# nvaccess/NVSpeechPlayer

Hardware: AMD Instinct MI355X
Metric: audio samples/sec (whole node) at 22.05 kHz Klatt synth, batch-N utterances (higher is better)
Workload: dtype f64

## Files before the change

nvspeechplayer_amd/csrc/klatt_batchplan.h:

```cpp
#pragma once

#include <stddef.h>
#include <stdint.h>

#include <algorithm>
#include <numeric>
#include <unordered_map>
#include <utility>
#include <vector>

#include "klatt_consts.h"

namespace klatt {


template <class Meta>
inline bool list_length(const Meta* meta, long long n, uint32_t& length)
{
    unsigned long long len = 0;
    for (long long k = 0; k < n; ++k) {
        const unsigned long long m = meta[k].minSamples, f = meta[k].fadeSamples;
        len += std::max(m, f + 1) + 1;
    }
    length = len >= 0xFFFFFFFFull ? 0u : (uint32_t)len;
    return len < 0xFFFFFFFFull;
}

template <class Meta>
inline unsigned long long list_timing(const Meta* meta, long long n)
{
    unsigned long long h = 0x9E3779B97F4A7C15ull ^ (unsigned long long)n;
    for (long long k = 0; k < n; ++k) {
        h ^= ((unsigned long long)meta[k].minSamples << 32) ^ meta[k].fadeSamples ^ ((unsigned long long)(meta[k].flags & FRAME_NULL) << 63);
        h *= 0xFF51AFD7ED558CCDull; h ^= h >> 29;
    }
    return h;
}

template <class Meta, class Facts>
inline void classify_list(const Meta* meta, const Facts* facts, long long n, uint32_t& flags, unsigned char& shape)
{
    uint32_t fl = 0;
    for (long long k = 0; k < n; ++k)
        if (!(meta[k].flags & FRAME_NULL)) fl |= facts[k].flags;
    const bool finite = !(fl & FACT_NONFINITE), needsNoise = (fl & FACT_NOISE) || !finite;
    flags = needsNoise ? UTT_NEEDS_NOISE : (!(fl & FACT_NASAL) ? UTT_NO_NASAL : 0u);
    shape = finite ? (!(fl & FACT_UNBOUNDED) ? 3 : 1) : 0;
}


struct ListTable {
    std::vector<uint32_t> lens;
    std::vector<unsigned long long> timing;
    std::vector<uint32_t> flags;
    std::vector<unsigned char> shape;
    std::vector<uint32_t> weight;
    long long size() const { return (long long)flags.size(); }
    unsigned long long run_key(long long l) const { return timing[(size_t)l] ^ ((unsigned long long)lens[(size_t)l] * 0x9E3779B97F4A7C15ull); }
};

struct RouteOptions {
    int tracks = 1, direct = 1, layout = -1;
    bool fast = false;
    bool sortByLength = true;
    bool noTracks = false;
    int cus = 256;
    long long nFrames = 0;
    bool want_tracks() const { return tracks && !noTracks; }
    bool want_direct() const { return direct && layout != 0 && nFrames > 0 && nFrames < 0xFFFFFFFFll; }
    bool plans() const { return (want_tracks() || want_direct()) && nFrames > 0; }
};

constexpr long long kRunMin = 32;

struct RunShare {
    long long total = 0, inRuns = 0;
    std::unordered_map<unsigned long long, long long> runOf;
};
template <class Pred>
inline RunShare run_share(const ListTable& lists, Pred pred)
{
    RunShare s;
    for (long long l = 0; l < lists.size(); ++l)
        if (pred(l)) { s.total += lists.weight[(size_t)l]; s.runOf[lists.run_key(l)] += lists.weight[(size_t)l]; }
    for (const auto& kv : s.runOf) if (kv.second >= kRunMin) s.inRuns += kv.second;
    return s;
}

using Rerouted = std::vector<std::pair<long long, uint32_t>>;
inline Rerouted reroute_lonely_quiet(ListTable& lists, const RouteOptions& o)
{
    Rerouted rerouted;
    if (!o.plans() || o.layout != -1) return rerouted;
    auto quiet = [&](long long l) { return !(lists.flags[(size_t)l] & UTT_NEEDS_NOISE); };
    const RunShare runs = run_share(lists, quiet);
    if (runs.runOf.size() <= 1) return rerouted;
    for (long long l = 0; l < lists.size(); ++l)
        if (quiet(l) && runs.runOf.at(lists.run_key(l)) < kRunMin) {
            rerouted.emplace_back(l, lists.flags[(size_t)l]);
            lists.flags[(size_t)l] = (lists.flags[(size_t)l] | UTT_NEEDS_NOISE) & ~UTT_NO_NASAL;
        }
    return rerouted;
}

inline std::vector<unsigned char> eligible_lists(const ListTable& lists, const RouteOptions& o)
{
    std::vector<unsigned char> eligible;
    if (!o.plans()) return eligible;
    eligible.assign((size_t)lists.size(), 0);
    for (long long l = 0; l < lists.size(); ++l)
        if ((lists.flags[(size_t)l] & UTT_NEEDS_NOISE) && lists.weight[(size_t)l]) eligible[(size_t)l] = lists.shape[(size_t)l];
    return eligible;
}

inline bool tracks_pay(const ListTable& lists, const unsigned char* eligible, const unsigned char* tracked, unsigned long long trackBytes, const RouteOptions& o)
{
    if (!(o.want_direct() && o.direct == 1 && o.fast && trackBytes > (128ull << 20))) return true;
    long long direct = 0;
    const RunShare runs = run_share(lists, [&](long long l) { return tracked[l] != 0; });
    for (long long l = 0; l < lists.size(); ++l)
        if (tracked[l] && (eligible[l] & 2)) direct += lists.weight[(size_t)l];
    const long long groups = (runs.total + kLanes - 1) / kLanes;
    return !(o.sortByLength && runs.inRuns * 2 <= runs.total && direct == runs.total && groups > o.cus);
}

inline void mark_tracked(ListTable& lists, const unsigned char* tracked, const uint32_t* kinds)
{
    for (long long l = 0; l < lists.size(); ++l)
        if (tracked[l]) lists.flags[(size_t)l] |= UTT_TRACKED | (kinds[l] << kUttKindShift);
// ... 53 lines not shown
    const long long ext = width - tail;
    std::vector<uint32_t> rep((size_t)ext);
    for (long long j = 0; j < ext; ++j) rep[(size_t)j] = order[(size_t)(end - tail + j % tail)];
    order.insert(order.begin() + end, rep.begin(), rep.end());
    return ext;
}

inline void fill_sparse_wavefronts(std::vector<uint32_t>& order, long long begin, int width)
{
    const int sparse = width / 2;
    std::vector<uint32_t> live((size_t)sparse);
    for (long long w = begin; w + width <= (long long)order.size(); w += width) {
        int nLive = 0;
        for (int i = 0; i < width && nLive < sparse; ++i)
            if (order[(size_t)(w + i)] != kNoUtt) live[(size_t)nLive++] = order[(size_t)(w + i)];
        if (nLive == 0 || nLive >= sparse) continue;
        int next = 0;
        for (int i = 0; i < width; ++i)
            if (order[(size_t)(w + i)] == kNoUtt) { order[(size_t)(w + i)] = live[(size_t)next]; next = (next + 1) % nLive; }
    }
}

template <class FlagsOf>
inline LanePacking pack_lanes(long long nUtt, FlagsOf flagsOf, const uint32_t* lens, const unsigned long long* timing, bool sortByLength, int width = kLanes)
{
    LanePacking p;
    std::vector<uint32_t>& order = p.order;
    order.resize((size_t)nUtt);
    std::iota(order.begin(), order.end(), 0u);
    auto quietEnd = std::stable_partition(order.begin(), order.end(), [&](uint32_t x) { return !(flagsOf(x) & UTT_NEEDS_NOISE); });
    p.nQuiet = quietEnd - order.begin();
    auto noNasalEnd = std::stable_partition(order.begin(), quietEnd, [&](uint32_t x) { return (flagsOf(x) & UTT_NO_NASAL) != 0; });
    p.nNoNasal = noNasalEnd - order.begin();
    auto trackedEnd = std::stable_partition(quietEnd, order.end(), [&](uint32_t x) { return (flagsOf(x) & UTT_TRACKED) != 0; });
    p.nTrackedUtt = trackedEnd - quietEnd;
    p.nTracked = p.nTrackedUtt;
    auto directEnd = std::stable_partition(trackedEnd, order.end(), [&](uint32_t x) { return (flagsOf(x) & UTT_DIRECT) != 0; });
    p.nDirectSlots = directEnd - trackedEnd;
    const bool untrackedFollow = directEnd != order.end();
    if (sortByLength) {
        auto before = [&](uint32_t x, uint32_t y) { return lens[x] != lens[y] ? lens[x] > lens[y] : timing[x] < timing[y]; };
        std::stable_sort(order.begin(), noNasalEnd, before);
        std::stable_sort(noNasalEnd, quietEnd, before);
        std::stable_sort(quietEnd, trackedEnd, before);
        std::stable_sort(trackedEnd, directEnd, before);
        std::stable_sort(directEnd, order.end(), before);
        const uint32_t* const o = order.data();
        const size_t q = (size_t)p.nQuiet, t = q + (size_t)p.nTrackedUtt, d = t + (size_t)p.nDirectSlots;
        std::vector<uint32_t> tracked, direct(o + t, o + d), untracked;
        pad_runs(o + q, o + t, lens, timing, width, tracked);
        if (!tracked.empty() && t != order.size()) tracked.insert(tracked.end(), lanes_to_boundary(tracked.size(), width), kNoUtt);
        if (!direct.empty() && untrackedFollow) direct.insert(direct.end(), lanes_to_boundary(direct.size(), width), kNoUtt);
        pad_runs(o + d, o + order.size(), lens, timing, width, untracked);
        p.nTracked = (long long)tracked.size();
        p.nDirectSlots = (long long)direct.size();
        order.resize(q);
        order.insert(order.end(), tracked.begin(), tracked.end());
        order.insert(order.end(), direct.begin(), direct.end());
        order.insert(order.end(), untracked.begin(), untracked.end());
    } else if (p.nDirectSlots > 0 && (untrackedFollow || p.nTrackedUtt > 0)) {
        const size_t padT = p.nTrackedUtt > 0 ? lanes_to_boundary((size_t)p.nTrackedUtt, width) : 0;
        order.insert(order.begin() + p.nQuiet + p.nTrackedUtt, padT, kNoUtt);
        p.nTracked = p.nTrackedUtt + (long long)padT;
        if (untrackedFollow) {
            const size_t padD = lanes_to_boundary((size_t)p.nDirectSlots, width);
            order.insert(order.begin() + p.nQuiet + p.nTracked + p.nDirectSlots, padD, kNoUtt);
            p.nDirectSlots += (long long)padD;
        }
    }
    p.nNoNasalSlots = p.nNoNasal + fill_tail(order, 0, p.nNoNasal, width);
    p.nQuietSlots = p.nQuiet + (p.nNoNasalSlots - p.nNoNasal);
    p.nQuietSlots += fill_tail(order, p.nNoNasalSlots, p.nQuietSlots, width);
    const long long noisy = (long long)order.size() - p.nQuietSlots;
    if (noisy % width != 0) {
        const long long ext = width - noisy % width;
        const long long untracked = noisy - p.nTracked - p.nDirectSlots;
        if (untracked <= 0) { if (p.nDirectSlots > 0) p.nDirectSlots += ext; else p.nTracked += ext; }
        order.insert(order.end(), (size_t)ext, kNoUtt);
    }
    fill_sparse_wavefronts(order, p.nQuietSlots, width);
    return p;
}

}
```

nvspeechplayer_amd/csrc/klatt_consts.h:

```cpp
#pragma once

#include <stdint.h>

namespace klatt {

constexpr int kLanes = 64;

constexpr uint32_t FRAME_NULL = 1u;
constexpr uint32_t UTT_NEEDS_NOISE = 1u;
constexpr uint32_t UTT_NO_NASAL = 2u;
constexpr uint32_t UTT_TRACKED = 4u;
constexpr uint32_t UTT_DIRECT = 8u;
constexpr int kUttKindShift = 8;

constexpr uint32_t FACT_NOISE = 1u;
constexpr uint32_t FACT_NONFINITE = 2u;
constexpr uint32_t FACT_NASAL = 4u;
constexpr uint32_t FACT_UNBOUNDED = 8u;

}
```

nvspeechplayer_amd/csrc/klatt_device.h:

```cpp
#pragma once

#include <hip/hip_runtime.h>
#include <stdint.h>
#include <type_traits>

#include "klatt_consts.h"
#include "klatt_layout.h"
#include "klatt_math.h"

namespace klatt {

constexpr int kTile = 32;
constexpr int kTileStride = kTile * 2 + 8;
constexpr int kSlots = 45;
constexpr int kBlock = 16;
constexpr int kStateDoubles = 240;

constexpr int MODE_EXACT = 0;
constexpr int MODE_FAST = 1;

constexpr int kTrackStages = 4;
#ifndef KLATT_FLAT_LAYOUT
#define KLATT_FLAT_LAYOUT 2
#endif
__host__ __device__ constexpr uint32_t track_stage_kinds(int s)
{
    return KLATT_FLAT_LAYOUT == 2 ? (s == 0 ? 0xF04003u : s == 1 ? 0x0000FCu : s == 2 ? 0x01B000u : 0x0E0F00u)
                                  : (s == 0 ? 0xF00000u : s == 1 ? 0x00403Fu : s == 2 ? 0x01B0C0u : 0x0E0F00u);
}
__host__ __device__ constexpr uint32_t track_stage_entries(int s)
{
    return KLATT_FLAT_LAYOUT == 2 ? (s == 0 ? 8u : s == 1 ? 6u : s == 2 ? 4u : 7u) : (s == 0 ? 4u : s == 1 ? 8u : s == 2 ? 6u : 7u);
}
constexpr int kTrackAntiStage = KLATT_FLAT_LAYOUT == 2 ? 0 : 1;
__host__ __device__ inline uint32_t track_stage_slots(uint32_t mask, int s) { return (uint32_t)__builtin_popcount(mask & track_stage_kinds(s)) + (s == kTrackAntiStage ? (mask & 1u) : 0u); }
__host__ __device__ inline uint32_t track_part(uint32_t mask, uint32_t F, int s)
{
    uint32_t at = 0;
    for (int k = 0; k < s; ++k) at += track_stage_entries(k) + (F - 1u) * track_stage_slots(mask, k);
    return at;
}

struct DirectHdr {
    uint32_t fadeSamples;
    uint32_t span;
    uint32_t bits;
    uint32_t pad;
};
constexpr uint32_t kDirectBwShift = 8, kDirectClsShift = 14, kDirectAllBits = 0x3FFFFFFu;
constexpr int kDirectStages = 8;
#ifndef KLATT_DIRECT_FAST_LAYOUT
#define KLATT_DIRECT_FAST_LAYOUT 1
#endif
__host__ __device__ constexpr int direct_layout(int mode) { return mode == MODE_FAST ? KLATT_DIRECT_FAST_LAYOUT : 0; }
__host__ __device__ constexpr int direct_stage_res(int s, int L = 0)
{
    return L == 1 ? (s < 2 ? 0 : (s == 3 || s == 4) ? 3 : 2) : (s == 0 ? 0 : 2);
}
__host__ __device__ constexpr int direct_stage_gains(int s, int L = 0)
{
    return L == 1 ? (s == 0 ? 1 : s == 1 ? 3 : s == 2 ? 1 : s == 5 ? 2 : s == 6 ? 1 : s == 7 ? 2 : 0)
                  : (s == 0 ? 4 : s == 1 ? 1 : s == 5 ? 2 : s == 6 ? 1 : s == 7 ? 2 : 0);
}
__host__ __device__ constexpr int direct_stage_entries(int s, int L = 0) { return 4 * direct_stage_res(s, L) + 3 * direct_stage_gains(s, L); }
__host__ __device__ constexpr int direct_stage_first(int s, int L = 0) { int at = 0; for (int k = 0; k < s; ++k) at += direct_stage_entries(k, L); return at; }
constexpr int kDirectEntries = direct_stage_first(kDirectStages);
static_assert(direct_stage_first(kDirectStages, 1) == kDirectEntries, "both layouts hold the same kinds");
__host__ __device__ constexpr int direct_stage_kind(int s, int e, int L = 0)
{
    constexpr int k0[kDirectStages][4] = {{20, 21, 22, 23}, {0, 1, 14, -1}, {2, 3, -1, -1}, {4, 5, -1, -1}, {6, 7, -1, -1}, {8, 9, 17, 18}, {10, 11, 19, -1}, {12, 13, 15, 16}};
    constexpr int k1[kDirectStages][4] = {{20, -1, -1, -1}, {21, 22, 23, -1}, {0, 1, 14, -1}, {2, 3, 4, -1}, {5, 6, 7, -1}, {8, 9, 17, 18}, {10, 11, 19, -1}, {12, 13, 15, 16}};
    return L == 1 ? k1[s][e] : k0[s][e];
}

struct KernelArgs {
    const DirectHdr* directHdr;
    const double2* directRec;
    const uint32_t* directFirst;
    uint32_t nDirect;
    const FlatRef* flatRef;
    const SourceRef* sourceRef;
    uint32_t trackBytes;
    const double2* track;
    const double* frames;
    const FrameMeta* meta;
    const UttDesc* utt;
    const uint32_t* order;
    int16_t* pcm;
    UttResult* result;
    double* state;
    double* const* statePtrs;
    const uint32_t* control;
    long long nSlots;
    uint32_t maxSamples;
    uint32_t ringMask;
    int sampleRate;
    double sampleRateF;
    double invSampleRate;
    double negPiOverSr;
    double twoPiOverSr;
    unsigned long long* debug;
};

__device__ constexpr int kResF[kNumRes] = {13, 14, 12, 11, 10, 9, 8, 7, 25, 26, 27, 28, 29, 30};
__device__ constexpr int kResB[kNumRes] = {21, 22, 20, 19, 18, 17, 16, 15, 31, 32, 33, 34, 35, 36};
constexpr int kNumHot = 17;
__device__ constexpr int kHot[kNumHot] = {1, 2, 3, 4, 5, 6, 23, 24, 37, 38, 39, 40, 41, 42, 43, 44, 45};


__device__ __forceinline__ double div_by(double x, double b, double y)
{
    double q = x * y;
    double r = __builtin_fma(-b, q, x);
    return __builtin_fma(r, y, q);
}

__device__ __forceinline__ double frac_toward_zero(double x) { return x - __builtin_trunc(x); }

__device__ __forceinline__ double fade_value(double from, double to, double ratio)
{
    double v = from + ((to - from) * ratio);
    return (to != to) ? from : v;
}

__device__ __forceinline__ uint32_t mix32(uint32_t x)
{
    x ^= x >> 16; x *= 0x7FEB352Du; x ^= x >> 15; x *= 0x846CA68Bu; x ^= x >> 16;
    return x;
}
__device__ __forceinline__ uint32_t noise_key(uint32_t seed) { return mix32(seed ^ 0x9E3779B9u); }
__device__ __forceinline__ uint32_t noise_inc(uint32_t seed) { return (mix32(seed + 0x85EBCA6Bu) << 1) | 1u; }
constexpr uint32_t kNoiseA = 1664525u;
constexpr uint32_t kNoiseA2 = kNoiseA * kNoiseA;
__device__ __forceinline__ uint32_t noise_inc2(uint32_t inc) { return (kNoiseA + 1u) * inc; }
__device__ __forceinline__ uint32_t noise_step(uint32_t s, uint32_t inc) { return s * kNoiseA + inc; }
__device__ __forceinline__ uint32_t noise_step2(uint32_t s, uint32_t inc2) { return s * kNoiseA2 + inc2; }
__device__ __forceinline__ uint32_t noise_first(uint32_t key, uint32_t inc) { return noise_step(key, inc); }
__device__ __forceinline__ double noise_uniform(uint32_t s)
{
    const double r = (double)(s >> 1);
    return __builtin_fma(r, 0x1.00000002p-31, r * 0x1p-93);
}

template <int MODE>
__device__ __forceinline__ double dot3(double a, double x, double b, double y, double c, double z)
{
    if (MODE == MODE_FAST) return __builtin_fma(c, z, __builtin_fma(b, y, a * x));
    return a * x + b * y + c * z;
}

#ifdef KLATT_SIGNAL_F32
typedef float sig_t;
#else
typedef double sig_t;
#endif
template <int MODE>
__device__ __forceinline__ float dot3(float a, float x, float b, float y, float c, float z)
{
    return __builtin_fmaf(c, z, __builtin_fmaf(b, y, a * x));
}
__device__ __forceinline__ float fade_value(float from, float to, float ratio)
{
    float v = from + ((to - from) * ratio);
    return (to != to) ? from : v;
}

struct Coef { double a, b, c; };
enum { COEF_UNREDUCED = 0, COEF_QUADRANT_M1 = 1, COEF_UNKNOWN = 2 };
#ifndef KLATT_COLD_CALL
#define KLATT_COLD_CALL 2
#endif
struct RadCos { double rad, cs; };
#if KLATT_COLD_CALL
__device__ __attribute__((noinline)) RadCos exp_cos_reduced(double ex, double th)
{
    RadCos o;
#if KLATT_COLD_CALL == 1
    if (__builtin_fabs(ex) <= 700.0 && __builtin_fabs(th) <= 1.0e4) { o.rad = fast_exp(ex); o.cs = fast_cos(th); }
    else
#endif
    { o.rad = exp(ex); o.cs = cos(th); }
    return o;
}
#endif
// ... 451 lines not shown
```

nvspeechplayer_amd/csrc/klatt_engine.hip:

```cpp
#include "klatt_device.h"
#include "klatt_systolic.h"
#include "klatt_lanepipe.h"
#include "klatt_tracks.h"
#include "klatt_direct.h"
#include "klatt_plan.h"
#include "klatt_timeline.h"
#include "klatt_align.h"
#include "klatt_source.h"
#include "klatt_response.h"
#include "klatt_stems.h"
#include "klatt_spectrum.h"
#include "klatt_resample.h"
#include "klatt_convolve.h"
#include "klatt_filter.h"
#include "klatt_codec.h"
#include "klatt_lpc.h"
#include "klatt_tempo.h"
#include "klatt_mix.h"
#include "klatt_export.h"
#include "klatt_batchplan.h"
#include "klatt_hostpool.h"
#include "klatt_trackplan.h"
#include "klatt_live.h"

// ... 413 lines not shown
        return 0;
    };
    int rc;
    switch (mode) {
    case MODE_EXACT: rc = go(klatt_lanepipe<MODE_EXACT, CH, WPS>); break;
    case MODE_FAST: rc = go(klatt_lanepipe<MODE_FAST, CH, WPS>); break;
    default: set_error("unknown arithmetic mode %d", mode); return -1;
    }
    if (rc) return rc;
    HIP_TRY(hipGetLastError());
    return 0;
}

#ifndef KLATT_NOISY_CH
#define KLATT_NOISY_CH 8
#endif
struct GroupPlan { bool systolic; int chunk; };
GroupPlan plan_group(int layout, bool noisy, long long nUttBatch, long long nNoisyBatch, int cus)
{
    const long long groups = (nUttBatch + kLanes - 1) / kLanes + 1;
    GroupPlan p;
    p.systolic = layout != 0;
    (void)nNoisyBatch;
    p.chunk = noisy ? (groups <= cus ? 16 : 8)
                    : (groups <= cus ? 32 : 16);
    return p;
}

template <bool STREAM, bool NOISE>
int launch(const KernelArgs& a, int mode, long long nWaves, hipStream_t stream)
{
    if (nWaves <= 0) return 0;
    if (nWaves > 0x7FFFFFFF) { set_error("too many wavefronts: %lld", nWaves); return -1; }
    constexpr int ldsBytes = LdsLayout<STREAM>::kBytes;
    auto go = [&](auto kernel) -> int {
        if (ensure_lds_limit(reinterpret_cast<const void*>(kernel), ldsBytes)) return -1;
        hipLaunchKernelGGL(kernel, dim3((unsigned)nWaves), dim3(kLanes), ldsBytes, stream, a);
        return 0;
    };
    int rc;
    switch (mode) {
    case MODE_EXACT: rc = go(klatt_synthesize<MODE_EXACT, STREAM, NOISE>); break;
    case MODE_FAST: rc = go(klatt_synthesize<MODE_FAST, STREAM, NOISE>); break;
    default:
        set_error("unknown arithmetic mode %d", mode);
        return -1;
    }
    if (rc) return rc;
    HIP_TRY(hipGetLastError());
    return 0;
}

int pick_device(int device)
{
    int n = 0;
    hipError_t e = hipGetDeviceCount(&n);
    if (e != hipSuccess || n <= 0) {
        set_error_code(SPEECHPLAYER_ERR_NO_DEVICE);
        set_error("no HIP device available (%s); this engine has no CPU path", e == hipSuccess ? "count 0" : hipGetErrorString(e));
        return -1;
    }
    if (device < 0) {
        const char* env = getenv("SPEECHPLAYER_DEVICE");
        if (env) device = atoi(env);
        else if (hipGetDevice(&device) != hipSuccess) device = 0;
    }
    if (device >= n) { set_error("device %d out of range (%d devices)", device, n); return -1; }
    return device;
}

struct Batch {
    int sampleRate = 0;
    int device = 0;
    int mode = MODE_EXACT;
    int sortByLength = 1;
    int layout = -1;
    int cus = 256;
    hipStream_t stream = nullptr;
    int tracks = 1;
    long long trackBudgetMB = 4096;
    hipStream_t side[6] = {nullptr, nullptr, nullptr, nullptr, nullptr, nullptr};
    hipEvent_t forkEvent = nullptr, join[6] = {nullptr, nullptr, nullptr, nullptr, nullptr, nullptr};
    int quietLast = 1;
    long long nUtt = 0, nFrames = 0, nSlots = 0;
    long long nLists = 0, nFramesSpoken = 0;
    std::vector<long long> uttFrameStart;
    std::vector<uint32_t> uttFrames;
    bool launched = false;
    long long nQuiet = 0;
    long long nTracked = 0;
    long long nTrackedUtt = 0;
    long long nJobs = 0, trackEntries = 0;
    int directLean = -1;
    bool directAligned = false;
    int direct = 1;
    long long nDirect = 0;
    long long nDirectUtt = 0, nDirectFrames = 0;
    long long nNoNasal = 0;
    long long nNoNasalUtt = 0;
    long long totalSamples = 0, poolSamples = 0;
    std::vector<uint32_t> lens;
    std::vector<uint32_t> uttSeed;
    std::vector<long long> outStart;
    std::vector<UttResult> results;
    bool resultsFresh = false;
    DeviceBuffer<double> dFrames;
    DeviceBuffer<FrameMeta> dMeta;
    DeviceBuffer<UttDesc> dUtt;
    DeviceBuffer<uint32_t> dOrder;
    DeviceBuffer<int16_t> dPcm;
    DeviceBuffer<UttResult> dResult;
    DeviceBuffer<FlatRef> dFlatRef;
    DeviceBuffer<SourceRef> dSourceRef;
    DeviceBuffer<TrackJob> dJobs;
    DeviceBuffer<double> dShapes;
    DeviceBuffer<double2> dTrack;
    DeviceBuffer<DirectJob> dDirectJobs;
    DeviceBuffer<uint32_t> dDirectFirst;
    DeviceBuffer<DirectHdr> dDirectHdr;
    DeviceBuffer<double2> dDirectRec;
    DeviceBuffer<unsigned long long> dDebug;
    DeviceBuffer<float> dFloat;
    DeviceBuffer<unsigned long long> dDigest;
    PinnedPair bounce;
    DeviceBuffer<FrameRecord> dRecords;
    DeviceBuffer<double> dShapeTable;
    DeviceBuffer<uint32_t> dRep;
    DeviceBuffer<unsigned long long> dMismatch;
    DeviceBuffer<FrameFacts> dFacts;
    PinnedBlock hFacts;
    DeviceBuffer<int16_t> dDense;
    DeviceBuffer<long long> dDenseStart;
    std::vector<long long> denseStart;
    hipStream_t copyStream = nullptr;
    hipEvent_t denseReady = nullptr, copyDone = nullptr;
    bool copyPending = false;
    bool floatFresh = false;
    hipEvent_t inputReady = nullptr;
    DeviceBuffer<long long> dShapeIdx;
    DeviceBuffer<double> dShapeRows;
    hipEvent_t pcmReady = nullptr;
    struct ExportSlot { PinnedBlock host; DeviceBuffer<unsigned char> dev; hipEvent_t done = nullptr; bool used = false; };
    static constexpr int kExportSlots = 16;
    ExportSlot exportSlot[kExportSlots];
    unsigned exportNext = 0;
    struct SharedTable {
        hipEvent_t done = nullptr;
        bool used = false;
        int wait(hipStream_t st) { if (used) HIP_TRY(hipStreamWaitEvent(st, done, 0)); return 0; }
        int mark(hipStream_t st) { HIP_TRY(hipEventRecord(done, st)); used = true; return 0; }
    };
    std::vector<uint32_t> uttList;
    DeviceBuffer<long long> dListStart;
    DeviceBuffer<TimelineReq> dTimeline;
    hipEvent_t setDone = nullptr, setCopied = nullptr, timelineReady = nullptr;
    bool timelineFresh = false;
    ExportSlot trackSlot[kExportSlots];
    unsigned trackNext = 0;
    DeviceBuffer<double> dPitch;
    SharedTable pitchOrder;
    long long pitchBudgetMB = 256;
    DeviceBuffer<FrameLabel> dLabels;
    DeviceBuffer<uint32_t> dUnitFirst;
    std::vector<uint32_t> listUnits;
    bool hasLabels = false;
    DeviceBuffer<double> dSource;
// ... 181 lines not shown
constexpr bool kTimingOnlyBuild = false;
#endif
bool refuse_timing_only(const char* what)
{
    if (!kTimingOnlyBuild || getenv("SPEECHPLAYER_ALLOW_TIMING_ONLY_PCM")) return false;
    set_error_code(SPEECHPLAYER_ERR_ARGUMENT);
    set_error("%s: this library was built with a timing-only experiment switch; its PCM is not valid", what);
    return true;
}

long long tracked_count(const Batch* b) { return (b->tracks && b->layout != 0) ? b->nTracked : 0; }
long long direct_count(const Batch* b) { return b->nDirect; }
bool direct_lean(const Batch* b, long long nGroups)
{
    if (b->directLean >= 0) return b->directLean != 0;
    if (b->directAligned) return false;
    return b->mode == MODE_FAST ? true : nGroups > 2ll * b->cus;
}

int batch_launch(Batch* b)
{
    KernelArgs a = base_args(b->sampleRate);
    a.frames = b->dFrames.ptr; a.meta = b->dMeta.ptr; a.utt = b->dUtt.ptr;
    a.pcm = b->dPcm.ptr; a.result = b->dResult.ptr; a.state = nullptr; a.control = nullptr;
    if (wait_exports(b)) return -1;
    b->resultsFresh = false;
    b->floatFresh = false;
    b->launched = true;
#ifdef KLATT_STAMPS
    if (b->dDebug.reserve((size_t)(b->nSlots / kLpUPG + 2) * 32 * 2)) return -1;
    HIP_TRY(hipMemsetAsync(b->dDebug.ptr, 0, b->dDebug.cap * 8, b->stream));
    a.debug = b->dDebug.ptr;
#endif
    const long long nLp = lanepipe_count(b);
    const bool laneKernel = b->layout == 0;
    const long long nTr = tracked_count(b);
    const long long nDir = direct_count(b);
    const long long nNoisyHead = b->nTracked - nTr;
    const long long nNoisy = b->nSlots - b->nQuiet - b->nTracked - nDir;
    const long long nNn = laneKernel ? 0 : b->nNoNasal - nLp;
    const long long nQ = b->nQuiet - nLp - nNn;
    const int parts = (nLp > 0) + (nNn > 0) + (nQ > 0) + (nNoisy > 0) + (nNoisyHead > 0) + (nTr > 0) + (nDir > 0);
    const bool fork = parts > 1;
    if (fork) HIP_TRY(hipEventRecord(b->forkEvent, b->stream));
    int sideUsed = 0, seen = 0;
    auto next_stream = [&](bool = false) -> hipStream_t {
        if (!fork || ++seen == parts) return b->stream;
        hipStream_t st = b->side[sideUsed++];
        (void)hipStreamWaitEvent(st, b->forkEvent, 0);
        return st;
    };
    const GroupPlan plq = plan_group(b->layout, false, b->nSlots, nNoisy, b->cus);
    auto launch_quiet = [&]() -> int {
    if (nLp > 0) {
        hipStream_t st = next_stream(true);
        a.order = b->dOrder.ptr; a.nSlots = nLp;
        const long long g = (nLp + kLpUPG - 1) / kLpUPG;
        if (g <= b->cus ? launch_lanepipe<KLATT_LP_CH, 1>(a, b->mode, g, st) : launch_lanepipe<16, 2>(a, b->mode, g, st)) return -1;
    }
    if (nNn > 0) {
        hipStream_t st = next_stream(true);
        a.order = b->dOrder.ptr + nLp; a.nSlots = nNn;
        const long long g = (nNn + kLanes - 1) / kLanes;
        if (plq.chunk == 32 ? launch_systolic<false, 32, 1, false>(a, b->mode, g, st) : launch_systolic<false, 16, 2, false>(a, b->mode, g, st)) return -1;
    }
    if (nQ > 0) {
        hipStream_t st = next_stream(true);
        a.order = b->dOrder.ptr + nLp + nNn; a.nSlots = nQ;
        const long long g = (nQ + kLanes - 1) / kLanes;
        if (plq.systolic ? (plq.chunk == 32 ? launch_systolic<false, 32>(a, b->mode, g, st) : launch_systolic<false, 16>(a, b->mode, g, st))
                         : launch<false, false>(a, b->mode, g, st)) return -1;
    }
        return 0;
    };
    const bool quietLast = b->quietLast && (nTr > 0 || nDir > 0) && nNoisy == 0 && nNoisyHead == 0;
    if (!quietLast && launch_quiet()) return -1;
    if (nTr > 0) {
        hipStream_t st = next_stream();
        TrackArgs t;
        t.jobs = b->dJobs.ptr; t.nJobs = b->nJobs; t.shapes = b->dShapes.ptr; t.track = b->dTrack.ptr;
        t.negPiOverSr = a.negPiOverSr; t.twoPiOverSr = a.twoPiOverSr;
        const long long tg = b->nJobs;
        if (tg > 0x7FFFFFFF) { set_error("too many tracks: %lld", b->nJobs); return -1; }
        hipLaunchKernelGGL(klatt_tracks, dim3((unsigned)tg), dim3(kLanes * kTrackWaves), 0, st, t);
        HIP_TRY(hipGetLastError());
        a.order = b->dOrder.ptr + b->nQuiet; a.nSlots = nTr;
        a.flatRef = b->dFlatRef.ptr; a.sourceRef = b->dSourceRef.ptr; a.track = b->dTrack.ptr;
        a.trackBytes = (uint32_t)std::min<unsigned long long>(((unsigned long long)b->trackEntries + kTrackPad) * sizeof(double2), 0xFFFFFFFFull);
        const GroupPlan pl = plan_group(b->layout, true, b->nSlots, nTr + nNoisy, b->cus);
        const long long g = (nTr + kLanes - 1) / kLanes;
        if (pl.chunk == 8 ? launch_systolic<true, KLATT_FLAT_CH, KLATT_FLAT_WPS, true, false, true>(a, b->mode, g, st)
                          : launch_systolic<true, 16, 1, true, false, true>(a, b->mode, g, st)) return -1;
        a.flatRef = nullptr; a.sourceRef = nullptr; a.track = nullptr;
    }
    if (nDir > 0) {
        hipStream_t st = next_stream();
        SeedArgs sa;
        sa.jobs = b->dDirectJobs.ptr; sa.nJobs = (uint32_t)b->nDirectFrames; sa.frames = b->dFrames.ptr; sa.meta = b->dMeta.ptr;
        sa.hdr = b->dDirectHdr.ptr; sa.rec = b->dDirectRec.ptr; sa.negPiOverSr = a.negPiOverSr; sa.twoPiOverSr = a.twoPiOverSr;
        const dim3 sg((unsigned)((b->nDirectFrames + 255) / 256), (unsigned)kDirectStages);
        constexpr int kSeedLds = 14 * 257 * (int)sizeof(double2);
        if (b->mode == MODE_FAST) hipLaunchKernelGGL(klatt_seeds<MODE_FAST>, sg, dim3(256), kSeedLds, st, sa);
        else hipLaunchKernelGGL(klatt_seeds<MODE_EXACT>, sg, dim3(256), kSeedLds, st, sa);
        HIP_TRY(hipGetLastError());
        a.order = b->dOrder.ptr + b->nQuiet + b->nTracked; a.nSlots = nDir;
        a.directHdr = b->dDirectHdr.ptr; a.directRec = b->dDirectRec.ptr; a.directFirst = b->dDirectFirst.ptr; a.nDirect = (uint32_t)b->nDirectFrames;
        a.sourceRef = b->dSourceRef.ptr;
        const long long g = (nDir + kLanes - 1) / kLanes;
        if (launch_direct(a, b->mode, direct_lean(b, g), g, st)) return -1;
        a.directHdr = nullptr; a.directRec = nullptr; a.directFirst = nullptr; a.nDirect = 0; a.sourceRef = nullptr;
    }
    for (int half = 0; half < 2; ++half) {
        const long long n = half ? nNoisy : nNoisyHead;
        if (n <= 0) continue;
        hipStream_t st = next_stream();
        a.order = b->dOrder.ptr + b->nQuiet + (half ? b->nTracked + nDir : 0); a.nSlots = n;
        const GroupPlan pl = plan_group(b->layout, true, b->nSlots, nTr + nNoisy + nNoisyHead, b->cus);
        const long long g = (n + kLanes - 1) / kLanes;
        if (pl.systolic ? (pl.chunk == 8 ? launch_systolic<true, KLATT_NOISY_CH, 2>(a, b->mode, g, st) : launch_systolic<true, 16>(a, b->mode, g, st))
                        : launch<false, true>(a, b->mode, g, st)) return -1;
    }
    if (quietLast && launch_quiet()) return -1;
    for (int i = 0; i < sideUsed; ++i) {
        HIP_TRY(hipEventRecord(b->join[i], b->side[i]));
        HIP_TRY(hipStreamWaitEvent(b->stream, b->join[i], 0));
    }
    return 0;
}

constexpr size_t kLogEntries = 40960;
constexpr size_t kLogEager = 2560;

struct LogEntry {
    double p[kNumParams];
    FrameMeta meta;
    uint32_t target;
    uint32_t pad;
};
static_assert(sizeof(LogEntry) == 400, "LogEntry layout");

__global__ void __launch_bounds__(256) live_scatter(const LogEntry* __restrict__ log, uint32_t n, double* __restrict__ ringFrames,
                                                    FrameMeta* __restrict__ ringMeta)
{
    const uint32_t e = blockIdx.x * 4u + (threadIdx.x >> 6), j = threadIdx.x & 63u;
    if (e >= n) return;
    const uint32_t at = log[e].target;
    if (at == kNoTarget) return;
    if (j < (uint32_t)kNumParams) ringFrames[(size_t)at * kNumParams + j] = log[e].p[j];
    else if (j == (uint32_t)kNumParams) ringMeta[at] = log[e].meta;
}

struct LivePlace {
    FrameMeta meta;
    long long row;
    uint32_t target;
    uint32_t pad;
};
static_assert(sizeof(LivePlace) == 32, "LivePlace layout");

__global__ void __launch_bounds__(256) live_place(const double* __restrict__ frames, const LivePlace* __restrict__ place, long long n,
                                                  double* __restrict__ ringFrames, FrameMeta* __restrict__ ringMeta)
{
    const uint32_t j = threadIdx.x & 63u;
    const long long step = (long long)gridDim.x * 4;
    for (long long e = (long long)blockIdx.x * 4 + (threadIdx.x >> 6); e < n; e += step) {
        const LivePlace p = place[e];
        if (j < (uint32_t)kNumParams) ringFrames[(size_t)p.target * kNumParams + j] = p.row < 0 ? 0.0 : frames[p.row * kNumParams + j];
        else if (j == (uint32_t)kNumParams) ringMeta[p.target] = p.meta;
    }
}

struct Stream {
    int sampleRate = 0;
    int device = 0;
    int mode = MODE_EXACT;
    uint32_t seed = 0;
// ... 858 lines not shown
    begin_call();
    QueueCall q;
    q.what = "speechPlayer_queueFramesManyDevice"; q.handles = handles; q.n = nHandles; q.frameStart = frameStart; q.frames = deviceFrames;
    q.onDevice = true; q.minDur = minFrameDuration; q.fadeDur = fadeDuration; q.userIndex = userIndex; q.isNull = isNull; q.purge = purge;
    q.readyStream = static_cast<hipStream_t>(readyStream);
    return queue_frames(q);
}

int speechPlayer_handleDevice(speechPlayer_handle_t handle)
{
    begin_call();
    Stream* s = lookup(handle);
    if (!s) { set_error("speechPlayer_handleDevice: invalid handle"); return -1; }
    return s->device;
}

speechPlayer_batch_t speechPlayer_batch_create(int sampleRate, int device)
{
    begin_call();
    int dev = pick_device(device);
    if (dev < 0) return nullptr;
    Batch* b = new Batch;
    b->sampleRate = sampleRate;
    b->device = dev;
    { hipDeviceProp_t prop; if (hipGetDeviceProperties(&prop, dev) == hipSuccess && prop.multiProcessorCount > 0) b->cus = prop.multiProcessorCount; }
    bool ok = hipSetDevice(dev) == hipSuccess && hipStreamCreateWithFlags(&b->stream, hipStreamNonBlocking) == hipSuccess &&
              hipEventCreateWithFlags(&b->forkEvent, hipEventDisableTiming) == hipSuccess &&
              hipStreamCreateWithFlags(&b->copyStream, hipStreamNonBlocking) == hipSuccess &&
              hipEventCreateWithFlags(&b->denseReady, hipEventDisableTiming) == hipSuccess &&
              hipEventCreateWithFlags(&b->copyDone, hipEventDisableTiming) == hipSuccess &&
              hipEventCreateWithFlags(&b->inputReady, hipEventDisableTiming) == hipSuccess &&
              hipEventCreateWithFlags(&b->pcmReady, hipEventDisableTiming) == hipSuccess;
    for (auto& s : b->exportSlot) ok = ok && hipEventCreateWithFlags(&s.done, hipEventDisableTiming) == hipSuccess;
    for (auto& s : b->trackSlot) ok = ok && hipEventCreateWithFlags(&s.done, hipEventDisableTiming) == hipSuccess;
    for (hipEvent_t* e : {&b->setDone, &b->setCopied, &b->timelineReady, &b->pitchOrder.done, &b->sourceOrder.done, &b->resampleOrder.done, &b->bankOrder.done}) ok = ok && hipEventCreateWithFlags(e, hipEventDisableTiming) == hipSuccess;
    { const char* e = getenv("SPEECHPLAYER_TRACKS"); if (e) b->tracks = atoi(e) ? 1 : 0; }
    { const char* e = getenv("SPEECHPLAYER_DIRECT"); if (e) b->direct = std::min(2, std::max(0, atoi(e))); }
    { const char* e = getenv("SPEECHPLAYER_DIRECT_LEAN"); if (e) b->directLean = std::min(1, std::max(-1, atoi(e))); }
    for (int i = 0; i < 6 && ok; ++i)
        ok = hipStreamCreateWithFlags(&b->side[i], hipStreamNonBlocking) == hipSuccess &&
             hipEventCreateWithFlags(&b->join[i], hipEventDisableTiming) == hipSuccess;
    { const char* e = getenv("SPEECHPLAYER_QUIET_LAST"); if (e) b->quietLast = atoi(e) ? 1 : 0; }
    if (!ok) {
        set_error("cannot create a stream on device %d", dev);
        speechPlayer_batch_destroy(b);
        return nullptr;
    }
    return b;
}

void speechPlayer_batch_destroy(speechPlayer_batch_t batch)
{
    Batch* b = static_cast<Batch*>(batch);
    if (!b) return;
    (void)hipSetDevice(b->device);
    (void)sync_exports(b);
    for (auto& s : b->exportSlot) {
        if (s.done) (void)hipEventDestroy(s.done);
        s.host.release(); s.dev.release();
    }
    (void)settle_track_exports(b, true);
    for (auto& s : b->trackSlot) {
        if (s.done) (void)hipEventDestroy(s.done);
        s.host.release(); s.dev.release();
    }
    for (hipEvent_t e : {b->setDone, b->setCopied, b->timelineReady, b->pitchOrder.done, b->sourceOrder.done, b->resampleOrder.done, b->bankOrder.done}) if (e) (void)hipEventDestroy(e);
    b->dListStart.release(); b->dTimeline.release(); b->dPitch.release(); b->dLabels.release(); b->dUnitFirst.release();
    b->dSource.release(); b->dEpochs.release(); b->dEpochCount.release(); b->dResample.release(); b->dBank.release();
    if (b->inputReady) (void)hipEventDestroy(b->inputReady);
    if (b->pcmReady) (void)hipEventDestroy(b->pcmReady);
    b->dShapeIdx.release(); b->dShapeRows.release();
    if (b->stream) { (void)hipStreamSynchronize(b->stream); (void)hipStreamDestroy(b->stream); }
    for (int i = 0; i < 6; ++i) {
        if (b->side[i]) { (void)hipStreamSynchronize(b->side[i]); (void)hipStreamDestroy(b->side[i]); }
        if (b->join[i]) (void)hipEventDestroy(b->join[i]);
    }
    if (b->forkEvent) (void)hipEventDestroy(b->forkEvent);
    if (b->copyStream) { (void)hipStreamSynchronize(b->copyStream); (void)hipStreamDestroy(b->copyStream); }
    if (b->denseReady) (void)hipEventDestroy(b->denseReady);
    if (b->copyDone) (void)hipEventDestroy(b->copyDone);
    b->dDense.release(); b->dDenseStart.release(); b->dFacts.release(); b->hFacts.release();
    b->dRecords.release(); b->dShapeTable.release(); b->dRep.release(); b->dMismatch.release();
    b->dFrames.release(); b->dMeta.release(); b->dUtt.release(); b->dOrder.release(); b->dPcm.release(); b->dResult.release();
    b->dFloat.release(); b->dDebug.release(); b->dDigest.release(); b->bounce.release();
    b->dFlatRef.release(); b->dSourceRef.release(); b->dJobs.release(); b->dShapes.release(); b->dTrack.release();
    b->dDirectJobs.release(); b->dDirectFirst.release(); b->dDirectHdr.release(); b->dDirectRec.release();
    delete b;
}

int speechPlayer_batch_setOption(speechPlayer_batch_t batch, const char* name, int value)
{
    begin_call();
    Batch* b = static_cast<Batch*>(batch);
    if (!b || !name) return -1;
    if (!strcmp(name, "mode")) {
        if (value != MODE_EXACT && value != MODE_FAST) { set_error("mode %d not available", value); return -1; }
        b->mode = value;
        return 0;
    }
    if (!strcmp(name, "sort")) { b->sortByLength = value ? 1 : 0; return 0; }
    if (!strcmp(name, "quiet_last")) { b->quietLast = value ? 1 : 0; return 0; }
    if (!strcmp(name, "layout")) { b->layout = value < 0 ? -1 : (value > 2 ? 1 : value); return 0; }
    if (!strcmp(name, "tracks")) { b->tracks = value ? 1 : 0; return 0; }
    if (!strcmp(name, "track_budget_mb")) { b->trackBudgetMB = value < 0 ? 0 : value; return 0; }
    if (!strcmp(name, "direct")) { b->direct = value < 0 ? 0 : (value > 2 ? 2 : value); return 0; }
    if (!strcmp(name, "direct_lean")) { b->directLean = value < 0 ? -1 : (value ? 1 : 0); return 0; }
    if (!strcmp(name, "pitch_table_mb")) { b->pitchBudgetMB = value < 1 ? 1 : value; return 0; }
    if (!strcmp(name, "source_table_mb")) { b->sourceBudgetMB = value < 1 ? 1 : value; return 0; }
    if (!strcmp(name, "source_lane_lists")) { b->sourceLaneLists = value < 1 ? 1 : value; return 0; }
    set_error("unknown option %s", name);
    return -1;
}

struct SetInput {
    long long nLists = 0;
    const long long* listStart = nullptr;
    const speechPlayer_frame_t* frames = nullptr;
    const unsigned int* minDur = nullptr;
    const unsigned int* fadeDur = nullptr;
    const int* userIndex = nullptr;
    const unsigned char* isNull = nullptr;
    const speechPlayer_frameRecord_t* records = nullptr;
    long long nShapes = 0;
    const speechPlayer_frame_t* shapes = nullptr;
    long long nUtt = 0;
    const unsigned int* listOf = nullptr;
    const unsigned int* seeds = nullptr;
    const double* deviceFrames = nullptr;
    hipStream_t readyStream = nullptr;
    const speechPlayer_frameLabel_t* labels = nullptr;
    bool noTracks = false;
};
static_assert(sizeof(speechPlayer_frameRecord_t) == sizeof(FrameRecord), "record layout");
static_assert(sizeof(speechPlayer_frameLabel_t) == sizeof(FrameLabel), "label layout");
static_assert(SPEECHPLAYER_LABEL_GAP == kLabelGap && SPEECHPLAYER_LABEL_PUFF == kLabelPuff && SPEECHPLAYER_ALIGN_COLUMNS == kAlignColumns &&
              SPEECHPLAYER_UNIT_COLUMNS == kUnitColumns, "alignment constants");

static void batch_clear(Batch* b)
{
    b->nUtt = 0; b->nFrames = 0; b->nFramesSpoken = 0; b->nLists = 0; b->nSlots = 0; b->nQuiet = 0; b->nNoNasal = 0; b->nNoNasalUtt = 0; b->totalSamples = 0; b->poolSamples = 0;
    b->nTracked = 0; b->nTrackedUtt = 0; b->nJobs = 0; b->trackEntries = 0; b->nDirect = 0; b->nDirectUtt = 0; b->nDirectFrames = 0; b->directAligned = false;
    b->lens.clear(); b->outStart.assign(1, 0); b->results.clear(); b->resultsFresh = false; b->floatFresh = false;
    b->uttFrameStart.clear(); b->uttFrames.clear(); b->uttList.clear(); b->uttSeed.clear(); b->timelineFresh = false; b->epochFresh = false;
    b->hasLabels = false; b->listUnits.clear();
}

static int batch_set(Batch* b, const SetInput& in);

static int batch_set_guarded(const char* what, speechPlayer_batch_t batch, const SetInput& in)
{
    begin_call();
    try {
        return batch_set(static_cast<Batch*>(batch), in);
    } catch (const std::exception& e) {
        set_error("%s: %s", what, e.what());
        return -1;
    }
}

int speechPlayer_batch_setUtterances(speechPlayer_batch_t batch, long long nUtterances, const long long* frameStart,
                                     const speechPlayer_frame_t* frames, const unsigned int* minFrameDuration,
                                     const unsigned int* fadeDuration, const int* userIndex, const unsigned char* isNull,
                                     const unsigned int* noiseSeed)
{
    SetInput in;
    in.nLists = nUtterances; in.listStart = frameStart; in.frames = frames; in.minDur = minFrameDuration; in.fadeDur = fadeDuration;
    in.userIndex = userIndex; in.isNull = isNull; in.nUtt = nUtterances; in.seeds = noiseSeed;
    return batch_set_guarded("setUtterances", batch, in);
}

static bool device_range(const void* p, size_t bytes, int device, size_t align, const char* what)
{
    hipPointerAttribute_t a;
    if (hipPointerGetAttributes(&a, p) != hipSuccess) {
        (void)hipGetLastError();
        set_error("%s: %p is not memory the HIP runtime knows (host memory?)", what, p);
        return false;
    }
    if (a.type != hipMemoryTypeDevice) { set_error("%s: %p is not device memory (memory type %d)", what, p, (int)a.type); return false; }
    if (a.device != device) { set_error("%s: %p is memory of device %d, the batch's is %d", what, p, a.device, device); return false; }
    if (reinterpret_cast<uintptr_t>(p) % align) { set_error("%s: %p is not %zu-byte aligned", what, p, align); return false; }
    hipDeviceptr_t base = nullptr;
    size_t size = 0;
    if (hipMemGetAddressRange(&base, &size, const_cast<void*>(p)) != hipSuccess) {
        (void)hipGetLastError();
        set_error("%s: the allocation that holds %p is unknown to the HIP runtime", what, p);
// ... 482 lines not shown
}

static int set_upload(SetCall& c)
{
    Batch* const b = c.b;
    const SetInput& in = c.in;
    const long long nL = c.nL, nU = c.nU, nF = c.nF, pool = c.pool, nSlotsAll = (long long)c.lanes.order.size();
    const long long nTrackedUtt = c.lanes.nTrackedUtt, nDirectUtt = c.nDirectUtt;
    const TrackPlan& plan = c.plan;
    const RawVector<DirectJob>& directJobs = c.scratch.directJobs;
    if ((size_t)pool > b->dPcm.cap && sync_exports(b)) return -1;
    if (b->dFrames.reserve(std::max<size_t>((size_t)nF * kNumParams, 1)) || b->dMeta.reserve(std::max<size_t>(nF, 1)) ||
        b->dUtt.reserve(std::max<size_t>(nU, 1)) || b->dOrder.reserve(std::max<size_t>(nSlotsAll, 1)) ||
        b->dResult.reserve(std::max<size_t>(nU, 1)) || b->dPcm.reserve(std::max<size_t>(pool, 1)) || b->dListStart.reserve((size_t)nL + 1))
        return -1;
    HIP_TRY(hipMemcpyAsync(b->dListStart.ptr, c.listStart, ((size_t)nL + 1) * sizeof(long long), hipMemcpyHostToDevice, b->stream));
    if (nTrackedUtt > 0) {
        if (b->dFlatRef.reserve((size_t)nF) || b->dJobs.reserve(plan.jobs.size()) || b->dShapes.reserve(plan.shapes.size()) ||
            b->dTrack.reserve((size_t)plan.entries + kTrackPad)) return -1;
        HIP_TRY(hipMemcpyAsync(b->dShapes.ptr, plan.shapes.data(), plan.shapes.size() * sizeof(double), hipMemcpyHostToDevice, b->stream));
        HIP_TRY(hipMemcpyAsync(b->dFlatRef.ptr, c.scratch.flatRef.data(), (size_t)nF * sizeof(FlatRef), hipMemcpyHostToDevice, b->stream));
        HIP_TRY(hipMemcpyAsync(b->dJobs.ptr, plan.jobs.data(), plan.jobs.size() * sizeof(TrackJob), hipMemcpyHostToDevice, b->stream));
    }
    if (nTrackedUtt > 0 || nDirectUtt > 0) {
        if (b->dSourceRef.reserve((size_t)nF)) return -1;
    }
    if (nDirectUtt > 0) {
        const size_t nD = directJobs.size();
        if (b->dDirectJobs.reserve(nD) || b->dDirectFirst.reserve((size_t)nU) || b->dDirectHdr.reserve((size_t)kDirectStages * nD) ||
            b->dDirectRec.reserve((size_t)kDirectEntries * nD)) return -1;
        HIP_TRY(hipMemcpyAsync(b->dDirectJobs.ptr, directJobs.data(), nD * sizeof(DirectJob), hipMemcpyHostToDevice, b->stream));
        HIP_TRY(hipMemcpyAsync(b->dDirectFirst.ptr, c.directFirst.data(), (size_t)nU * sizeof(uint32_t), hipMemcpyHostToDevice, b->stream));
    }
    if (nF) {
        if (!c.earlyStarted) HIP_TRY(hipMemcpyAsync(b->dFrames.ptr, in.frames, (size_t)nF * kNumParams * sizeof(double), hipMemcpyHostToDevice, b->stream));
        if (!c.byRecords) HIP_TRY(hipMemcpyAsync(b->dMeta.ptr, c.scratch.meta.data(), (size_t)nF * sizeof(FrameMeta), hipMemcpyHostToDevice, b->stream));
    }
    if (nU) {
        HIP_TRY(hipMemcpyAsync(b->dUtt.ptr, c.utt.data(), (size_t)nU * sizeof(UttDesc), hipMemcpyHostToDevice, b->stream));
        HIP_TRY(hipMemcpyAsync(b->dOrder.ptr, c.lanes.order.data(), (size_t)nSlotsAll * sizeof(uint32_t), hipMemcpyHostToDevice, b->stream));
        HIP_TRY(hipMemsetAsync(b->dResult.ptr, 0, (size_t)nU * sizeof(UttResult), b->stream));
        if (b->dDenseStart.reserve((size_t)nU + 1)) return -1;
        HIP_TRY(hipMemcpyAsync(b->dDenseStart.ptr, c.denseStart.data(), ((size_t)nU + 1) * sizeof(long long), hipMemcpyHostToDevice, b->stream));
    }
    if (c.verify) {
        if (b->dRep.reserve((size_t)nF) || b->dMismatch.reserve(1)) return -1;
        HIP_TRY(hipMemcpyAsync(b->dRep.ptr, plan.rep.data(), (size_t)nF * sizeof(uint32_t), hipMemcpyHostToDevice, b->stream));
        HIP_TRY(hipMemsetAsync(b->dMismatch.ptr, 0xFF, sizeof(unsigned long long), b->stream));
    }
    if (in.labels) {
        if (b->dLabels.reserve(std::max<size_t>((size_t)nF, 1)) || b->dUnitFirst.reserve(std::max<size_t>((size_t)(nF + nL), 1))) return -1;
        c.copyGuard.armed = true;
        if (nF) HIP_TRY(hipMemcpyAsync(b->dLabels.ptr, in.labels, (size_t)nF * sizeof(FrameLabel), hipMemcpyHostToDevice, b->copyStream));
        if (nF + nL) HIP_TRY(hipMemcpyAsync(b->dUnitFirst.ptr, c.unitFirst.data(), (size_t)(nF + nL) * sizeof(uint32_t), hipMemcpyHostToDevice, b->copyStream));
    }
    HIP_TRY(hipStreamSynchronize(b->stream));
    if (c.copyGuard.armed) { HIP_TRY(hipStreamSynchronize(b->copyStream)); c.copyGuard.armed = false; }
    if (c.early.joinable()) c.early.join();
    if (c.earlyRc) { set_error_code(SPEECHPLAYER_ERR_HIP); set_error("set: uploading the frames failed: %s", c.earlyErr.c_str()); return -1; }
    const unsigned grid = (unsigned)std::min<long long>((nF + 255) / 256, 1 << 16);
    if (c.verify) {
        hipLaunchKernelGGL(klatt_verify_shared, dim3(grid), dim3(256), 0, b->stream, b->dFrames.ptr, b->dRep.ptr, nF, b->dMismatch.ptr);
        HIP_TRY(hipGetLastError());
        HIP_TRY(hipMemcpyAsync(&c.mismatchAt, b->dMismatch.ptr, sizeof c.mismatchAt, hipMemcpyDeviceToHost, b->stream));
    }
    if (nTrackedUtt > 0 || nDirectUtt > 0) {
        hipLaunchKernelGGL(klatt_source_refs, dim3(grid), dim3(256), 0, b->stream, b->dFrames.ptr, b->dMeta.ptr, b->dSourceRef.ptr, nF);
        HIP_TRY(hipGetLastError());
    }
    if (c.verify || nTrackedUtt > 0 || nDirectUtt > 0) HIP_TRY(hipStreamSynchronize(b->stream));
    return 0;
}

static int set_commit(SetCall& c)
{
    Batch* const b = c.b;
    const LanePacking& lanes = c.lanes;
    b->hasLabels = c.in.labels != nullptr;
    b->listUnits.swap(c.listUnits);
    b->nUtt = c.nU; b->nFrames = c.nF; b->nFramesSpoken = c.spoken; b->nLists = c.nL; b->nSlots = (long long)lanes.order.size();
    b->nNoNasalUtt = lanes.nNoNasal;
    b->nQuiet = lanes.nQuietSlots; b->nNoNasal = lanes.nNoNasalSlots;
    b->nTracked = lanes.nTrackedUtt > 0 ? lanes.nTracked : 0; b->nTrackedUtt = lanes.nTrackedUtt;
    b->nJobs = lanes.nTrackedUtt > 0 ? (long long)c.plan.jobs.size() : 0; b->trackEntries = lanes.nTrackedUtt > 0 ? (long long)c.plan.entries : 0;
    b->nDirect = c.nDirectUtt > 0 ? lanes.nDirectSlots : 0; b->nDirectUtt = c.nDirectUtt; b->nDirectFrames = (long long)c.scratch.directJobs.size();
    b->directAligned = c.nDirectUtt > 0 && c.directAligned;
    b->totalSamples = c.total; b->poolSamples = c.pool;
    b->lens.swap(c.lens); b->outStart.swap(c.outStart); b->denseStart.swap(c.denseStart);
    b->uttFrameStart.swap(c.uttFrameStart); b->uttFrames.swap(c.uttFrames); b->uttList.swap(c.uttList); b->uttSeed.swap(c.uttSeed);
    b->timelineFresh = false; b->epochFresh = false;
    HIP_TRY(hipEventRecord(b->setDone, b->stream));
    HIP_TRY(hipEventRecord(b->setCopied, b->copyStream));
    b->results.clear();
    b->resultsFresh = false;
    b->floatFresh = false;
    b->launched = false;
    return 0;
}

static int batch_set(Batch* b, const SetInput& in)
{
    if (!b || in.nLists < 0 || in.nUtt < 0 || !in.listStart) { set_error("set: bad arguments"); return -1; }
    if (in.nUtt >= 0xFFFFFFFFll || in.nLists >= 0xFFFFFFFFll) { set_error("set: too many utterances"); return -1; }
    if (!in.listOf && in.nUtt != in.nLists) { set_error("set: %lld utterances for %lld lists and no listOf", in.nUtt, in.nLists); return -1; }
    SetCall c(b, in);
    HIP_TRY(hipSetDevice(b->device));
    if (set_validate(c) || set_meta_words(c)) return -1;
    if (set_start_frames(c) || set_frame_facts(c) || set_plan(c)) return -1;
    set_direct_jobs_and_refs(c);
    set_lanes(c);
    c.verify = !c.byRecords && c.lanes.nTrackedUtt > 0 && !c.plan.rep.empty();
    if (set_upload(c)) {
        batch_clear(b);
        return -1;
    }
    c.lap("uploads");
    if (c.verify && c.mismatchAt != ~0ull) {
        const unsigned long long k = c.mismatchAt;
        if (c.early.joinable()) c.early.join();
        SetInput again = in;
        again.noTracks = true;
        const uint32_t first = c.plan.rep[(size_t)k];
        const int rc = batch_set(b, again);
        if (rc == 0) {
            set_error("set: frames %llu and %u carry one 128-bit shape hash and different values; the batch runs without tracks", k, first);
            set_error_code(SPEECHPLAYER_OK);
        }
        return rc;
    }
    return set_commit(c);
}

long long speechPlayer_batch_frames(speechPlayer_batch_t batch, long long u, speechPlayer_frame_t* frames, unsigned int* minFrameDuration,
                                    unsigned int* fadeDuration, int* userIndex, unsigned char* isNull, long long capacity)
{
    begin_call();
    Batch* b = static_cast<Batch*>(batch);
    if (!b || u < 0 || u >= b->nUtt) { set_error("batch_frames: no such utterance"); return -1; }
    HIP_TRY(hipSetDevice(b->device));
    const long long n = b->uttFrames[(size_t)u], k0 = b->uttFrameStart[(size_t)u];
    if (n > capacity || n == 0) return n;
    if (frames) HIP_TRY(hipMemcpy(frames, b->dFrames.ptr + k0 * kNumParams, (size_t)n * sizeof(speechPlayer_frame_t), hipMemcpyDeviceToHost));
    if (minFrameDuration || fadeDuration || userIndex || isNull) {
        std::vector<FrameMeta> m((size_t)n);
        HIP_TRY(hipMemcpy(m.data(), b->dMeta.ptr + k0, (size_t)n * sizeof(FrameMeta), hipMemcpyDeviceToHost));
        for (long long k = 0; k < n; ++k) {
            if (minFrameDuration) minFrameDuration[k] = m[(size_t)k].minSamples;
            if (fadeDuration) fadeDuration[k] = m[(size_t)k].fadeSamples;
            if (userIndex) userIndex[k] = m[(size_t)k].userIndex;
            if (isNull) isNull[k] = (m[(size_t)k].flags & FRAME_NULL) ? 1 : 0;
        }
    }
    return n;
}

long long speechPlayer_batch_utteranceSamples(speechPlayer_batch_t batch, long long u)
{
    Batch* b = static_cast<Batch*>(batch);
    if (!b || u < 0 || u >= b->nUtt) return -1;
    return b->lens[u];
}
long long speechPlayer_batch_lengths(speechPlayer_batch_t batch, long long* lengths, long long capacity)
{
    begin_call();
    Batch* b = static_cast<Batch*>(batch);
    if (!b) { set_error("batch_lengths: no batch"); return -1; }
// ... 657 lines not shown
    if (!b || !out) return -1;
    int n = (int)std::min<size_t>(b->dDebug.cap, (size_t)capacity);
    if (n > 0) HIP_TRY(hipMemcpy(out, b->dDebug.ptr, (size_t)n * 8, hipMemcpyDeviceToHost));
    return n;
}

int speechPlayer_batch_kernelInfo(speechPlayer_batch_t batch, int* info, int nInfo)
{
    begin_call();
    Batch* b = static_cast<Batch*>(batch);
    if (!b || !info || nInfo < 6) return -1;
    HIP_TRY(hipSetDevice(b->device));
    hipFuncAttributes fa;
    const long long nNoisy = b->nSlots - b->nQuiet, nLp = lanepipe_count(b);
    const long long nNn = b->layout == 0 ? 0 : b->nNoNasal - nLp, nQ = b->nQuiet - nLp - nNn;
    const bool lanepipe = nLp > 0 && nLp >= nQ && nLp >= nNoisy && nLp >= nNn;
    const bool nasalFree = !lanepipe && nNn > 0 && nNn >= nQ && nNn >= nNoisy;
    const bool noisy = !lanepipe && !nasalFree && nNoisy >= nQ;
    const GroupPlan pl = plan_group(b->layout, noisy, b->nSlots, nNoisy, b->cus);
    const bool fast = b->mode == MODE_FAST;
    const long long nTr = tracked_count(b);
    const long long nDir = direct_count(b);
    const bool directG = noisy && nDir > 0 && nDir >= nTr && nDir >= nNoisy - nTr - nDir;
    const bool tracked = noisy && !directG && nTr > 0 && nTr >= nNoisy - nTr - nDir;
    const void* fn;
    int ldsBytes = LdsLayout<false>::kBytes, chunk = 0, wavesPerGroup = 1;
    long long groups = (nNn + kLanes - 1) / kLanes + (nQ + kLanes - 1) / kLanes + (nNoisy + kLanes - 1) / kLanes;
    if (nasalFree) {
        if (pl.chunk == 32) { fn = fast ? (const void*)klatt_systolic<MODE_FAST, false, 32, 1, false> : (const void*)klatt_systolic<MODE_EXACT, false, 32, 1, false>; ldsBytes = SysLds<false, 32>::kBytes; }
        else { fn = fast ? (const void*)klatt_systolic<MODE_FAST, false, 16, 2, false> : (const void*)klatt_systolic<MODE_EXACT, false, 16, 2, false>; ldsBytes = SysLds<false, 16>::kBytes; }
        chunk = pl.chunk;
        wavesPerGroup = kStages;
    } else if (lanepipe) {
        const long long g = (nLp + kLpUPG - 1) / kLpUPG;
        if (g <= b->cus) { fn = fast ? (const void*)klatt_lanepipe<MODE_FAST, KLATT_LP_CH, 1> : (const void*)klatt_lanepipe<MODE_EXACT, KLATT_LP_CH, 1>; ldsBytes = LpLds<KLATT_LP_CH>::kBytes; chunk = KLATT_LP_CH; }
        else { fn = fast ? (const void*)klatt_lanepipe<MODE_FAST, 16, 2> : (const void*)klatt_lanepipe<MODE_EXACT, 16, 2>; ldsBytes = LpLds<16>::kBytes; chunk = 16; }
        wavesPerGroup = kStages;
        groups = g;
    } else if (directG) {
        if (direct_lean(b, (nDir + kLanes - 1) / kLanes)) {
            fn = fast ? (const void*)klatt_direct<MODE_FAST, kDirectLeanChunk, 4> : (const void*)klatt_direct<MODE_EXACT, kDirectLeanChunk, 4>;
            ldsBytes = DirectLds<kDirectLeanChunk>::kBytes; chunk = kDirectLeanChunk;
        } else {
            fn = fast ? (const void*)klatt_direct<MODE_FAST, kDirectChunk, 2> : (const void*)klatt_direct<MODE_EXACT, kDirectChunk, 2>;
            ldsBytes = DirectLds<kDirectChunk>::kBytes; chunk = kDirectChunk;
        }
        wavesPerGroup = kDirectStages;
    } else if (tracked) {
        if (pl.chunk == 8) { fn = fast ? (const void*)klatt_systolic<MODE_FAST, true, KLATT_FLAT_CH, KLATT_FLAT_WPS, true, false, true> : (const void*)klatt_systolic<MODE_EXACT, true, KLATT_FLAT_CH, KLATT_FLAT_WPS, true, false, true>; ldsBytes = SysLds<true, KLATT_FLAT_CH, true>::kBytes; chunk = KLATT_FLAT_CH; }
        else { fn = fast ? (const void*)klatt_systolic<MODE_FAST, true, 16, 1, true, false, true> : (const void*)klatt_systolic<MODE_EXACT, true, 16, 1, true, false, true>; ldsBytes = SysLds<true, 16, true>::kBytes; chunk = 16; }
        wavesPerGroup = kStages;
    } else if (pl.systolic) {
        if (noisy && pl.chunk == 8) { fn = fast ? (const void*)klatt_systolic<MODE_FAST, true, 8, 2> : (const void*)klatt_systolic<MODE_EXACT, true, 8, 2>; ldsBytes = SysLds<true, 8>::kBytes; }
        else if (noisy) { fn = fast ? (const void*)klatt_systolic<MODE_FAST, true, 16> : (const void*)klatt_systolic<MODE_EXACT, true, 16>; ldsBytes = SysLds<true, 16>::kBytes; }
        else if (pl.chunk == 32) { fn = fast ? (const void*)klatt_systolic<MODE_FAST, false, 32> : (const void*)klatt_systolic<MODE_EXACT, false, 32>; ldsBytes = SysLds<false, 32>::kBytes; }
        else { fn = fast ? (const void*)klatt_systolic<MODE_FAST, false, 16> : (const void*)klatt_systolic<MODE_EXACT, false, 16>; ldsBytes = SysLds<false, 16>::kBytes; }
        chunk = pl.chunk;
        wavesPerGroup = kStages;
    } else {
        fn = fast ? (noisy ? (const void*)klatt_synthesize<MODE_FAST, false, true> : (const void*)klatt_synthesize<MODE_FAST, false, false>)
                  : (noisy ? (const void*)klatt_synthesize<MODE_EXACT, false, true> : (const void*)klatt_synthesize<MODE_EXACT, false, false>);
    }
    HIP_TRY(hipFuncGetAttributes(&fa, fn));
    hipDeviceProp_t prop;
    HIP_TRY(hipGetDeviceProperties(&prop, b->device));
    info[0] = fa.numRegs;
    info[1] = ldsBytes;
    info[2] = (int)(groups * wavesPerGroup);
    info[3] = prop.multiProcessorCount;
    info[4] = (int)(prop.sharedMemPerMultiprocessor / ldsBytes);
    info[5] = (int)fa.localSizeBytes;
    if (nInfo >= 8) { info[6] = chunk; info[7] = noisy ? 1 : 0; }
    if (nInfo >= 10) { info[8] = lanepipe ? 1 : 0; info[9] = (int)std::min<long long>(nLp > 0 ? b->nNoNasalUtt : 0, 0x7FFFFFFF); }
    if (nInfo >= 12) { info[10] = nasalFree ? 1 : 0; info[11] = (int)std::min<long long>(nNn > 0 ? b->nNoNasalUtt : 0, 0x7FFFFFFF); }
    if (nInfo >= 16) {
        info[12] = (int)std::min<long long>(nTr > 0 ? b->nTrackedUtt : 0, 0x7FFFFFFF); info[13] = (int)std::min<long long>(b->nJobs, 0x7FFFFFFF);
        info[14] = (int)std::min<long long>(b->trackEntries * (long long)sizeof(double2) >> 20, 0x7FFFFFFF); info[15] = tracked ? 1 : 0;
    }
    if (nInfo >= 20) {
        info[16] = (int)std::min<long long>(b->nDirectUtt, 0x7FFFFFFF); info[17] = directG ? 1 : 0;
        info[18] = (int)std::min<long long>(b->nDirectFrames * (long long)(kDirectEntries * sizeof(double2) + kDirectStages * sizeof(DirectHdr)) >> 20, 0x7FFFFFFF);
        info[19] = 0;
    }
    return 0;
}


static long long plan_tracks_view(long long nUtterances, const long long* frameStart, const speechPlayer_frame_t* frames,
                                  const unsigned int* fadeDuration, const unsigned char* isNull, const unsigned char* eligible,
                                  long long budgetMB, const void* facts24, unsigned long long* trackOff, unsigned int* trackMask, unsigned char* tracked,
                                  unsigned long long* nEntries, long long* collisionAt, unsigned int* kinds = nullptr)
{
    begin_call();
    if (nUtterances < 0 || !frameStart || frameStart[0] != 0) { set_error("planTracks: bad arguments"); return -1; }
    for (long long u = 0; u < nUtterances; ++u)
        if (frameStart[u + 1] < frameStart[u]) { set_error("planTracks: frameStart not monotone at %lld", u); return -1; }
    const long long nF = frameStart[nUtterances];
    if (nF > 0 && (!frames || !fadeDuration)) { set_error("planTracks: bad frame arrays"); return -1; }
    std::vector<FrameMeta> meta((size_t)nF);
    for (long long k = 0; k < nF; ++k) {
        meta[k].minSamples = 0; meta[k].userIndex = -1;
        meta[k].fadeSamples = std::max(fadeDuration[k], 1u);
        meta[k].flags = (isNull && isNull[k]) ? FRAME_NULL : 0u;
    }
    std::vector<unsigned char> all;
    if (!eligible) { all.assign((size_t)nUtterances, 1); eligible = all.data(); }
    TrackPlan plan;
    std::vector<FrameFacts> own;
    const FrameFacts* facts = static_cast<const FrameFacts*>(facts24);
    if (!facts) {
        own.resize((size_t)nF);
        parallel_ranges(nF, 1 << 14, [&](long long a, long long e) { for (long long k = a; k < e; ++k) own[k] = frame_facts(reinterpret_cast<const double*>(frames + k), 1e300, 1e300); });
        facts = own.data();
    }
    plan_tracks(nUtterances, frameStart, FrameSource{frames, nullptr, nullptr}, facts, meta.data(), eligible, track_budget_entries(budgetMB), plan_hash_mask(), plan);
    if (collisionAt) *collisionAt = -1;
    for (long long k = 0; k < nF && !plan.rep.empty(); ++k) {
        const uint32_t r = plan.rep[(size_t)k];
        if (r == 0xFFFFFFFFu || (long long)r == k) continue;
        if (!shape_values_equal(reinterpret_cast<const double*>(frames + k), reinterpret_cast<const double*>(frames + r))) {
            if (collisionAt) *collisionAt = k;
            set_error("planTracks: frames %lld and %u carry one 128-bit shape hash and different values", k, r);
            return -2;
        }
    }
    for (long long k = 0; k < nF; ++k) {
        if (trackOff) trackOff[k] = plan.ref[k].off;
        if (trackMask) trackMask[k] = plan.ref[k].mask;
    }
    for (long long u = 0; u < nUtterances; ++u) {
        if (tracked) tracked[u] = plan.tracked[u];
        if (kinds) kinds[u] = plan.tracked[u] ? plan.kinds[u] : 0u;
        if (!plan.tracked[u])
            for (long long k = frameStart[u]; k < frameStart[u + 1]; ++k) { if (trackOff) trackOff[k] = 0; if (trackMask) trackMask[k] = 0; }
    }
    if (nEntries) *nEntries = plan.entries;
    return (long long)plan.jobs.size();
}

long long speechPlayer_planTracks(long long nUtterances, const long long* frameStart, const speechPlayer_frame_t* frames,
                                  const unsigned int* fadeDuration, const unsigned char* isNull, const unsigned char* eligible,
                                  long long budgetMB, unsigned long long* trackOff, unsigned int* trackMask, unsigned char* tracked,
                                  unsigned long long* nEntries)
{
    try {
        return plan_tracks_view(nUtterances, frameStart, frames, fadeDuration, isNull, eligible, budgetMB, nullptr, trackOff, trackMask, tracked, nEntries, nullptr);
    } catch (const std::exception& e) { set_error("planTracks: %s", e.what()); return -1; }
}

long long speechPlayer_planTracksFacts(long long nUtterances, const long long* frameStart, const speechPlayer_frame_t* frames,
                                       const unsigned int* fadeDuration, const unsigned char* isNull, const unsigned char* eligible,
                                       long long budgetMB, const void* facts24, unsigned long long* trackOff, unsigned int* trackMask,
                                       unsigned char* tracked, unsigned long long* nEntries, long long* collisionAt)
{
    try {
        return plan_tracks_view(nUtterances, frameStart, frames, fadeDuration, isNull, eligible, budgetMB, facts24, trackOff, trackMask, tracked, nEntries, collisionAt);
    } catch (const std::exception& e) { set_error("planTracksFacts: %s", e.what()); return -1; }
}

long long speechPlayer_planTrackKinds(long long nUtterances, const long long* frameStart, const speechPlayer_frame_t* frames,
                                      const unsigned int* fadeDuration, const unsigned char* isNull, const unsigned char* eligible,
                                      long long budgetMB, unsigned long long* trackOff, unsigned int* trackMask, unsigned char* tracked,
                                      unsigned long long* nEntries, unsigned int* kinds)
{
    try {
        return plan_tracks_view(nUtterances, frameStart, frames, fadeDuration, isNull, eligible, budgetMB, nullptr, trackOff, trackMask, tracked, nEntries, nullptr, kinds);
    } catch (const std::exception& e) { set_error("planTrackKinds: %s", e.what()); return -1; }
}

void speechPlayer_internal_parallel(long long n, long long grain, void (*fn)(void* ctx, long long a, long long e), void* ctx)
{
    if (n <= 0 || !fn) return;
    parallel_ranges(n, grain, [&](long long a, long long e) { fn(ctx, a, e); });
}

long long speechPlayer_frameFacts(const speechPlayer_frame_t* frames, long long nFrames, int sampleRate, int onDevice, void* facts24)
{
    begin_call();
    if (nFrames < 0 || (nFrames > 0 && (!frames || !facts24)) || sampleRate <= 0) { set_error("frameFacts: bad arguments"); return -1; }
    const double maxBw = 690.0 * sampleRate / M_PI, maxF = 9900.0 * sampleRate / (2.0 * M_PI);
    FrameFacts* const out = static_cast<FrameFacts*>(facts24);
    if (!onDevice) {
        parallel_ranges(nFrames, 1 << 13, [&](long long a, long long e) { for (long long k = a; k < e; ++k) out[k] = frame_facts(reinterpret_cast<const double*>(frames + k), maxF, maxBw); });
        return nFrames;
    }
    if (nFrames == 0) return 0;
    DeviceBuffer<double> dF;
    DeviceBuffer<FrameFacts> dO;
    struct Release { DeviceBuffer<double>& a; DeviceBuffer<FrameFacts>& b; ~Release() { a.release(); b.release(); } } release{dF, dO};
    if (dF.reserve((size_t)nFrames * kNumParams) || dO.reserve((size_t)nFrames)) return -1;
    HIP_TRY(hipMemcpy(dF.ptr, frames, (size_t)nFrames * kNumParams * sizeof(double), hipMemcpyHostToDevice));
    const unsigned grid = (unsigned)std::min<long long>((nFrames + 255) / 256, 1 << 16);
    hipLaunchKernelGGL(klatt_frame_facts, dim3(grid), dim3(256), 0, nullptr, dF.ptr, dO.ptr, nFrames, maxF, maxBw);
    HIP_TRY(hipGetLastError());
    HIP_TRY(hipMemcpy(out, dO.ptr, (size_t)nFrames * sizeof(FrameFacts), hipMemcpyDeviceToHost));
    return nFrames;
}

long long speechPlayer_planDirect(long long nUtterances, const long long* frameStart, const unsigned char* isNull,
                                  unsigned int* from, unsigned int* to, unsigned int* flags)
{
    begin_call();
    if (nUtterances < 0 || !frameStart || frameStart[0] != 0) { set_error("planDirect: bad arguments"); return -1; }
    for (long long u = 0; u < nUtterances; ++u)
        if (frameStart[u + 1] < frameStart[u]) { set_error("planDirect: frameStart not monotone at %lld", u); return -1; }
    const long long nF = frameStart[nUtterances];
    if (nF >= 0xFFFFFFFFll) { set_error("planDirect: too many frames"); return -1; }
    std::vector<FrameMeta> meta((size_t)nF);
    for (long long k = 0; k < nF; ++k) { meta[k].minSamples = 0; meta[k].fadeSamples = 1; meta[k].userIndex = -1; meta[k].flags = (isNull && isNull[k]) ? FRAME_NULL : 0u; }
    std::vector<DirectJob> jobs;
    jobs.reserve((size_t)nF);
    for (long long u = 0; u < nUtterances; ++u) walk_fade_ends(frameStart[u], frameStart[u + 1], meta.data(), jobs);
    for (long long k = 0; k < nF; ++k) {
        if (from) from[k] = jobs[(size_t)k].from;
        if (to) to[k] = jobs[(size_t)k].to;
        if (flags) flags[k] = jobs[(size_t)k].flags;
    }
    return nF;
}

long long speechPlayer_planTimeline(long long nUtterances, const long long* frameStart, const unsigned int* minFrameDuration,
                                    const unsigned int* fadeDuration, long long* firstSample, long long* length)
{
    begin_call();
    if (nUtterances < 0 || !frameStart || frameStart[0] != 0) { set_error("planTimeline: bad arguments"); return -1; }
    for (long long u = 0; u < nUtterances; ++u)
        if (frameStart[u + 1] < frameStart[u]) { set_error("planTimeline: frameStart not monotone at %lld", u); return -1; }
    const long long nF = frameStart[nUtterances];
    if (nF > 0 && (!minFrameDuration || !fadeDuration)) { set_error("planTimeline: no durations"); return -1; }
    for (long long u = 0; u < nUtterances; ++u) {
        long long S = 0;
        for (long long k = frameStart[u]; k < frameStart[u + 1]; ++k) {
            if (firstSample) firstSample[k] = S;
            FrameMeta m;
            m.minSamples = minFrameDuration[k]; m.fadeSamples = std::max(fadeDuration[k], 1u);
            S += timeline_span(m);
        }
        if (length) length[u] = S;
    }
    return nF;
}

long long speechPlayer_batch_timeline(speechPlayer_batch_t batch, long long u, long long* firstSample, int* userIndex, long long capacity)
{
    begin_call();
    Batch* b = static_cast<Batch*>(batch);
    if (!b || u < 0 || u >= b->nUtt) { set_error("batch_timeline: no such utterance"); return -1; }
    HIP_TRY(hipSetDevice(b->device));
    const long long n = b->uttFrames[(size_t)u], k0 = b->uttFrameStart[(size_t)u];
    if (n > capacity || (!firstSample && !userIndex)) return n;
    std::vector<FrameMeta> m((size_t)n);
    if (n) HIP_TRY(hipMemcpy(m.data(), b->dMeta.ptr + k0, (size_t)n * sizeof(FrameMeta), hipMemcpyDeviceToHost));
    long long S = 0;
    for (long long k = 0; k < n; ++k) {
        if (firstSample) firstSample[k] = S;
        if (userIndex) userIndex[k] = m[(size_t)k].userIndex;
        S += timeline_span(m[(size_t)k]);
    }
    if (firstSample) firstSample[n] = S;
    return n;
}

static int export_output(Batch* b, const char* what, void* deviceOut, long long elements, size_t elSize)
{
    HIP_TRY(hipSetDevice(b->device));
    if (!deviceOut) { set_error("%s: no output buffer", what); return -1; }
    return device_range(deviceOut, (size_t)elements * elSize, b->device, elSize, what) ? 0 : -1;
}

static int export_synthesised(const Batch* b, const char* what)
{
    if (!b->launched) set_error("%s: the batch has not been synthesised since it was set", what);
    return b->launched ? 0 : -1;
}

static int step_request(const char* what, long long& hop, long long& phase, long long rowStride)
{
    if (hop <= 0 || phase < 0) { set_error("%s: hop %lld, phase %lld", what, hop, phase); return -1; }
// ... 2048 lines not shown
```

nvspeechplayer_amd/csrc/klatt_plan.h:

```cpp
#pragma once

#include <stdint.h>
#include <string.h>

#include "klatt_consts.h"
#include "klatt_layout.h"
#if defined(__HIPCC__)
#include "klatt_device.h"
#endif

namespace klatt {

struct FrameFacts {
    unsigned long long h0, h1;
    uint32_t flags;
    uint32_t pad;
};

KLATT_LAYOUT_HD inline bool fact_finite(double v)
{
    unsigned long long w;
    memcpy(&w, &v, 8);
    return (w & 0x7FF0000000000000ull) != 0x7FF0000000000000ull;
}
KLATT_LAYOUT_HD inline double fact_abs(double v) { return v < 0 ? -v : v; }
KLATT_LAYOUT_HD constexpr unsigned long long fact_key(int n)
{
    unsigned long long z = (unsigned long long)(n + 1) * 0x9E3779B97F4A7C15ull;
    z = (z ^ (z >> 30)) * 0xBF58476D1CE4E5B9ull;
    z = (z ^ (z >> 27)) * 0x94D049BB133111EBull;
    return z ^ (z >> 31);
}
KLATT_LAYOUT_HD inline unsigned long long fact_fold(unsigned long long a, unsigned long long c)
{
#if defined(__HIP_DEVICE_COMPILE__)
    return (__umul64hi(a, c) ^ (a * c)) + a + ((c << 32) | (c >> 32));
#else
    const unsigned __int128 m = (unsigned __int128)a * c;
    return ((unsigned long long)(m >> 64) ^ (unsigned long long)m) + a + ((c << 32) | (c >> 32));
#endif
}

KLATT_LAYOUT_HD inline uint32_t pitch_flags(double p0, double p46)
{
    uint32_t fl = 0;
    if (!fact_finite(p0) || !fact_finite(p46)) fl |= 2u;
    if (!(fact_abs(p0) <= 1e30) || !(fact_abs(p46) <= 1e30)) fl |= 4u;
    return fl;
}
KLATT_LAYOUT_HD inline uint32_t shape_flags(const double* p, double maxF, double maxBw)
{
    uint32_t fl = 0;
    if (p[3] != 0.0 || p[6] != 0.0 || p[24] != 0.0) fl |= 1u;
    bool finite = true;
    for (int i = 1; i < kNumParams - 1; ++i) finite = finite && fact_finite(p[i]);
    if (!finite) fl |= 2u;
    for (int i = 25; i <= 30; ++i)
        if (!(fact_abs(p[i]) <= 1e6) || !(p[i + 6] >= 0.0) || !(p[i + 6] <= 1e6)) fl |= 1u;
    if (p[23] != 0.0 || !(p[21] >= 1.0) || !(p[22] >= 0.0) || !(p[21] <= 1e6) || !(p[22] <= 1e6) ||
        !(fact_abs(p[13]) <= 1e6) || !(fact_abs(p[14]) <= 1e6) || !(fact_abs(p[5]) <= 1e30) || !(fact_abs(p[44]) <= 1e30))
        fl |= 4u;
    bool inRange = true;
    for (int i = 7; i <= 14; ++i) inRange = inRange && (fact_abs(p[i]) <= maxF) && (p[i + 8] >= 0.0) && (p[i + 8] <= maxBw);
    for (int i = 25; i <= 30; ++i) inRange = inRange && (fact_abs(p[i]) <= maxF) && (p[i + 6] >= 0.0) && (p[i + 6] <= maxBw);
    if (!inRange) fl |= 8u;
    return fl;
}
KLATT_LAYOUT_HD inline bool shape_values_equal(const double* a, const double* c)
{
    bool same = true;
    for (int i = 1; i < kNumParams - 1; ++i) {
        unsigned long long x, y;
        memcpy(&x, &a[i], 8); memcpy(&y, &c[i], 8);
        same = same && x == y;
    }
    return same;
}

KLATT_LAYOUT_HD inline FrameFacts frame_facts(const double* p, double maxF, double maxBw)
{
    FrameFacts o;
    const uint32_t fl = shape_flags(p, maxF, maxBw) | pitch_flags(p[0], p[46]);
    unsigned long long x = 0x9E3779B97F4A7C15ull, y = 0xC2B2AE3D27D4EB4Full;
#if defined(__HIPCC__)
#pragma unroll
#endif
    for (int i = 0; i < 46; i += 2) {
        unsigned long long w0, w1 = 0;
        memcpy(&w0, &p[1 + i], 8);
        if (i + 1 < kShapeValues) memcpy(&w1, &p[2 + i], 8);
        x ^= fact_fold(w0 ^ fact_key(2 * i), w1 ^ fact_key(2 * i + 1));
        y ^= fact_fold(w0 ^ fact_key(2 * i + 100), w1 ^ fact_key(2 * i + 101));
    }
    x ^= x >> 32; x *= 0xD6E8FEB86659FD93ull; x ^= x >> 32;
    y ^= y >> 31; y *= 0xBF58476D1CE4E5B9ull; y ^= y >> 29;
    o.h0 = x; o.h1 = y; o.flags = fl; o.pad = 0;
    return o;
}

#if defined(__HIPCC__)
__global__ void __launch_bounds__(256) klatt_frame_facts(const double* __restrict__ frames, FrameFacts* __restrict__ out, long long nFrames, double maxF, double maxBw)
{
    const long long stride = (long long)gridDim.x * blockDim.x;
    for (long long k = (long long)blockIdx.x * blockDim.x + threadIdx.x; k < nFrames; k += stride) {
        double p[kNumParams];
        const double* src = frames + k * kNumParams;
#pragma unroll
        for (int i = 0; i < kNumParams; ++i) p[i] = src[i];
        out[k] = frame_facts(p, maxF, maxBw);
    }
}

struct FrameRecord {
    double voicePitch, endVoicePitch;
    uint32_t shape;
    uint32_t minSamples, fadeSamples;
    int32_t userIndex;
};
constexpr uint32_t kRecordSilence = 0xFFFFFFFFu;
static_assert(sizeof(FrameRecord) == 32, "FrameRecord layout");

__global__ void __launch_bounds__(256) klatt_expand_frames(const FrameRecord* __restrict__ records, const double* __restrict__ shapes,
                                                           double* __restrict__ frames, FrameMeta* __restrict__ meta, long long nFrames)
{
    constexpr int kTileFrames = 64, kTilePairs = kTileFrames * kNumParams / 2;
    __shared__ FrameRecord rec[kTileFrames];
    const long long nTiles = (nFrames + kTileFrames - 1) / kTileFrames;
    for (long long tile = blockIdx.x; tile < nTiles; tile += gridDim.x) {
        const long long k0 = tile * kTileFrames;
        const int n = (int)((nFrames - k0) < (long long)kTileFrames ? (nFrames - k0) : (long long)kTileFrames);
        __syncthreads();
        if ((int)threadIdx.x < n) {
            const FrameRecord r = records[k0 + threadIdx.x];
            rec[threadIdx.x] = r;
            FrameMeta m;
            m.minSamples = r.minSamples;
            m.fadeSamples = r.fadeSamples > 1u ? r.fadeSamples : 1u;
            m.userIndex = r.userIndex;
            m.flags = r.shape == kRecordSilence ? FRAME_NULL : 0u;
            meta[k0 + threadIdx.x] = m;
        }
        __syncthreads();
        auto value = [&](int j) -> double {
            const int f = j / kNumParams, p = j - f * kNumParams;
// ... 30 lines not shown
```

nvspeechplayer_amd/csrc/klatt_systolic.h:

```cpp
#pragma once

#include <type_traits>

#include "klatt_device.h"

namespace klatt {

#ifndef KLATT_UNROLL
#define KLATT_UNROLL 8
#endif
#ifndef KLATT_MINWAVES
#define KLATT_MINWAVES 1
#endif
#ifndef KLATT_PAIR
#define KLATT_PAIR 1
#endif
#ifndef KLATT_NOISY_RUNS
#define KLATT_NOISY_RUNS 0
#endif
#ifndef KLATT_FADE_TIGHT
#define KLATT_FADE_TIGHT 1
#endif
#ifndef KLATT_NOISY_TIGHT
#define KLATT_NOISY_TIGHT 1
#endif
#define KLATT_STR2(x) #x
#define KLATT_STR(x) KLATT_STR2(x)

#ifndef KLATT_FLAT_EXHAUSTIVE
#define KLATT_FLAT_EXHAUSTIVE 1
#endif
constexpr int kStages = 4;
#ifndef KLATT_FLAT_SOURCE
#define KLATT_FLAT_SOURCE 1
#endif

template <bool NOISE, int CH, bool FLAT = false, int SPLIT = 0>
struct SysLds {
    static constexpr int MOVED = SPLIT & 3;
    static constexpr bool NP0 = (SPLIT >> 2) != 0;
    static constexpr int kBufs = 2;
    static constexpr int kBufsX = 2;
    static constexpr int kBufBytes = CH * kLanes * (FLAT ? (int)sizeof(sig_t) : 8);
    static constexpr int kPipeBytes = kBufs * kBufBytes;
    static constexpr int kNumPipes = NOISE ? 4 : 3;
    static constexpr int kPipeO = kBufsX * kBufBytes;
    static constexpr int kTileOff = kPipeO + (kNumPipes - 1) * kPipeBytes;
    static constexpr int kRowBase = kTileOff + kLanes * kTileStride;
    static constexpr int kRowCount = kRowBase + kLanes * 8;
    static constexpr int kMaxLen = kRowCount + kLanes * 4;
    static constexpr int kSync = kMaxLen + 16;
    static constexpr int kFrames = kSync + 32;
    static constexpr int kParams0 = (FLAT && KLATT_FLAT_SOURCE) ? 0 : (NP0 ? 12 : 7), kParams1 = FLAT ? 0 : (NOISE ? (NP0 ? 0 : 5) + 2 * (3 + MOVED) : 7), kParams2 = FLAT ? 0 : (NOISE ? 14 - 2 * MOVED : 6), kParams3 = FLAT ? 0 : (NOISE ? 14 : 5);
    static constexpr int kFrames1 = kFrames + 1 * kParams0 * kLanes * 8;
    static constexpr int kFrames2 = kFrames1 + 2 * kParams1 * kLanes * 8;
    static constexpr int kFrames3 = kFrames2 + 2 * kParams2 * kLanes * 8;
    static constexpr int kBytes = kFrames3 + 2 * kParams3 * kLanes * 8;
};

template <int NPARAM, int NRES, bool NWREG = false>
struct StageFrame {
    double* oldL;
    double* nwL;
    double nwR[NWREG && NPARAM > 0 ? NPARAM : 1];
    __device__ __forceinline__ double getNew(int k) const { return NWREG ? nwR[k] : nwL[k * kLanes]; }
    __device__ __forceinline__ void setNew(int k, double v) { if (NWREG) nwR[k] = v; else nwL[k * kLanes] = v; }
    double cur[NPARAM > 0 ? NPARAM : 1];
    double ra[NRES > 0 ? NRES : 1], rb[NRES > 0 ? NRES : 1], rc[NRES > 0 ? NRES : 1];
    double z1[NRES > 0 ? NRES : 1], z2[NRES > 0 ? NRES : 1];
    double invFade;
    uint32_t cnt, oldMin, newMin, newFade, nextFrame, resMask, parMask, produced;
    bool hasNew, oldNull, newNull, done;
};

struct PitchState {
    double cur0, old0, new0, oldInc, newInc;
};

template <int NPARAM, int NRES, bool NWREG>
__device__ __forceinline__ void stage_frame_init(StageFrame<NPARAM, NRES, NWREG>& f, bool live, unsigned char* region, int lane)
{
    f.oldL = reinterpret_cast<double*>(region) + lane;
    f.nwL = f.oldL + NPARAM * kLanes;
#pragma unroll
    for (int k = 0; k < NPARAM; ++k) { f.oldL[k * kLanes] = 0.0; f.setNew(k, 0.0); f.cur[k] = 0.0; }
#pragma unroll
    for (int r = 0; r < NRES; ++r) { f.ra[r] = 0.0; f.rb[r] = 2.0; f.rc[r] = -1.0; f.z1[r] = 0.0; f.z2[r] = 0.0; }
    f.invFade = 1.0;
    f.cnt = 0; f.oldMin = 0; f.newMin = 0; f.newFade = 1; f.nextFrame = 0; f.resMask = 0; f.parMask = 0; f.produced = 0;
    f.hasNew = false; f.oldNull = true; f.newNull = false; f.done = !live;
}

template <int NPARAM_, int NRES_, int GAIN_, bool PITCH_, bool ANTI0_, bool INLINE_COEF_ = false>
struct StageDesc {
    static constexpr int NPARAM = NPARAM_, NRES = NRES_, GAIN = GAIN_;
    static constexpr bool PITCH = PITCH_, ANTI0 = ANTI0_, INLINE_COEF = INLINE_COEF_;
};

struct StageCtx {
    const KernelArgs& A;
    const UttDesc& d;
    const double* myFrames;
    const FrameMeta* myMeta;
    uint32_t ringOff, ringMask;
    const FlatRef* myFlat;
    const SourceRef* mySrc;
    bool lone = false;
    double* loneLds = nullptr;
};
constexpr int kLoneLdsPerStage = 12288;
#ifndef KLATT_STREAM_SPLIT
#define KLATT_STREAM_SPLIT 5
#endif
#ifndef KLATT_LONE_SPLIT
#define KLATT_LONE_SPLIT 7
// ... 547 lines not shown
                        }
                    }
                    if (K::RUNS && !K::LONE && !forceGeneral()) {
                        const bool fad = f.hasNew;
                        const uint32_t rem = f.done ? 0xFFFFFFFFu : (fad ? f.newFade - f.cnt : (f.oldMin > f.cnt ? f.oldMin - f.cnt : 0u));
                        const bool anyFad = __any(!f.done && fad), anySteady = __any(!f.done && !fad);
                        int n = 0;
                        if (!(anyFad && anySteady) && !__any(!f.done && fad && f.cnt == 0u) && !(anyFad && nan_target_live(f))) {
                            const int cap = lim - i;
#pragma unroll
                            for (int st = CH; st >= 1; st >>= 1)
                                if (n + st <= cap && __all(rem >= (uint32_t)(n + st))) n += st;
                        }
                        if (n >= 2) {
                            int kr = anyFad ? 1 : 0;
                            bool lerpR = false, gainOnlyR = false;
                            uint32_t wResR = 0;
                            if (kr == 1) {
                                lerpR = __any(!f.done && f.parMask != 0u);
                                gainOnlyR = D::GAIN >= 0 && !__any(!f.done && (f.parMask & ~(1u << GI)) != 0u);
                                wResR = wave_or_bits<(D::NRES > 0 ? D::NRES : 1)>(f.done ? 0u : f.resMask);
                                if (!D::PITCH && !lerpR && wResR == 0u) kr = 0;
                            }
                            if (!f.done) {
                                if (kr == 0) {
#pragma nounroll
                                    for (int j = i; j < i + n; ++j) body(c, j, true, K::PRE ? preIn(c, j) : 0.0);
                                    f.cnt += (uint32_t)n;
                                    steadyDone(n);
                                } else {
#pragma nounroll
                                    for (int j = i; j < i + n; ++j) {
                                        f.cnt++;
                                        stage_fade<D, MODE, true>(f, ps, X.A, RF, RB, lerpR, wResR, gainOnlyR);
                                        body(c, j, false, 0.0);
                                    }
                                    fadeDone(n);
                                }
                            }
                            i += n;
                            continue;
                        }
                    }
                    if (K::DELAY) {
                        const bool hold = delay > 0u;
                        const bool wasDone = f.done;
                        if (hold) { delay--; f.done = true; }
                        const bool emit = stage_advance<D, MODE>(f, ps, lastIndex, P, RF, RB, X);
                        if (hold) f.done = wasDone;
                        gen(c, i, emit);
                    } else if (K::CACHE) {
                        if (!cached) {
#pragma unroll
                            for (int k = 0; k < D::NPARAM; ++k) { co[k] = f.oldL[k * kLanes]; cn[k] = f.getNew(k); }
                            cached = true;
                        }
                        bool anyEvent = false;
                        const bool emit = stage_advance<D, MODE>(f, ps, lastIndex, P, RF, RB, X, co, cn, &anyEvent);
                        if (anyEvent) cached = false;
                        gen(c, i, emit);
                    } else {
                        const bool emit = stage_advance<D, MODE>(f, ps, lastIndex, P, RF, RB, X);
                        if (K::LONE) loneValid = false;
                        gen(c, i, emit);
                    }
                    ++i;
                }
            }
            perChunk();
        }
        STAMP_WORKED();
        STAGE_SYNC();
        STAMP_SYNCED();
    }
#ifdef KLATT_STAMPS
    if (X.A.debug && (threadIdx.x & (kLanes - 1)) == 0) {
        unsigned long long* o = X.A.debug + (blockIdx.x * 4 + stampSlot) * 8;
        o[0] = st.work; o[1] = st.wait; o[2] = st.n[0]; o[3] = st.n[1]; o[4] = st.n[2]; o[5] = st.c[0]; o[6] = st.c[1]; o[7] = st.c[2];
    }
#endif
    (void)stampSlot;
}

template <int STAGE_, int NRES_, int NGAIN_, bool ANTI0_, uint32_t USUAL_ = 0, uint32_t USUAL2_ = 0, class R_ = sig_t>
struct FlatDesc {
    using R = R_;
    static constexpr int STAGE = STAGE_;
    static constexpr int NRES = NRES_, NGAIN = NGAIN_, NE = NRES_ + NGAIN_;
    static constexpr bool ANTI0 = ANTI0_;
    static constexpr uint32_t USUAL = USUAL_, USUAL2 = USUAL2_;
};

struct BarrierSync {
    __device__ __forceinline__ void begin(int) const {}
    __device__ __forceinline__ void end(int) const { __syncthreads(); }
    __device__ __forceinline__ void idle() const { __syncthreads(); }
};

#ifndef KLATT_MIX_UNROLL
#define KLATT_MIX_UNROLL 4
#endif
template <int E> using KindTag = std::integral_constant<int, E>;
typedef unsigned int flat_u4 __attribute__((ext_vector_type(4)));
typedef unsigned int flat_u2 __attribute__((ext_vector_type(2)));
typedef double flat_d2 __attribute__((ext_vector_type(2)));
template <class FD>
struct FlatState2 {
    static constexpr int NR = FD::NRES > 0 ? FD::NRES : 1;
    using R = typename FD::R;
    R ra[NR], rb[NR], rc[NR], z1[NR], z2[NR];
    R cur[2 * FD::NGAIN > 0 ? 2 * FD::NGAIN : 1];
    uint32_t idx[FD::NE], stride[FD::NE];
    uint32_t startAt, left, next, nFrames, length, produced;
    FlatRef nextRef;
    uint32_t wmask;
    bool live;
};
template <class R> struct ResPre { R a, p1, p2; };
template <class T> __device__ __forceinline__ void flat_pin(T v) { asm volatile("" :: "v"(v) : "memory"); }
template <class R> __device__ __forceinline__ void flat_pin(const ResPre<R>& q) { asm volatile("" :: "v"(q.a), "v"(q.p1), "v"(q.p2) : "memory"); }
template <int NE>
__device__ __forceinline__ uint32_t flat2_wave_kinds(uint32_t flags, bool live, const int* GE)
{
    const uint32_t mine = live ? (flags >> kUttKindShift) : 0u;
    uint32_t w = 0;
#pragma unroll
    for (int e = 0; e < NE; ++e) w |= __any((mine >> GE[e]) & 1u) ? (1u << e) : 0u;
    return w;
}
template <class FD>
__device__ __forceinline__ void flat2_init(FlatState2<FD>& f, bool live, const UttDesc& d, const StageCtx& X, const int* GE)
{
#pragma unroll
    for (int r = 0; r < FD::NRES; ++r) { f.ra[r] = 0; f.rb[r] = 2; f.rc[r] = -1; f.z1[r] = 0; f.z2[r] = 0; }
#pragma unroll
    for (int k = 0; k < 2 * FD::NGAIN; ++k) f.cur[k] = 0;
#pragma unroll
    for (int e = 0; e < FD::NE; ++e) { f.idx[e] = 0; f.stride[e] = 0; }
    f.live = live && d.length > 0u;
    f.nFrames = d.nFrames; f.length = d.length; f.next = 0; f.left = 0; f.produced = 0;
    const bool any = live && d.nFrames > 0u;
    f.startAt = any ? 1u : 0xFFFFFFFFu;
    f.nextRef = FlatRef{0u, 0u, 1u, 0u};
    if (any) f.nextRef = X.myFlat[0];
    f.wmask = (uint32_t)__builtin_amdgcn_readfirstlane((int)flat2_wave_kinds<FD::NE>(d.flags, live, GE));
}
template <class FD>
__device__ __forceinline__ void flat2_switch(FlatState2<FD>& f, const StageCtx& X, const int* GE)
{
    const FlatRef p = f.nextRef;
    const uint32_t part = p.off + track_part(p.mask, p.fadeSamples, FD::STAGE);
    const uint32_t nMove = track_stage_slots(p.mask, FD::STAGE), hdr = track_stage_entries(FD::STAGE) - nMove;
    uint32_t moving = 0, still = 0;
#pragma unroll
    for (int e = 0; e < FD::NE; ++e) {
        const bool moves = (p.mask >> GE[e]) & 1u;
        f.idx[e] = (part + (moves ? hdr + moving : still)) * 16u;
        f.stride[e] = moves ? nMove * 16u : 0u;
        const uint32_t w = GE[e] == 0 ? 2u : 1u;
        moving += moves ? w : 0u; still += moves ? 0u : w;
    }
    f.left = nMove ? p.fadeSamples : 1u;
    f.next++;
    const bool more = f.next < f.nFrames;
    f.startAt = more ? f.startAt + p.span : 0xFFFFFFFFu;
#pragma unroll
    for (int e = 0; e < FD::NE; ++e) { flat_pin(f.idx[e]); flat_pin(f.stride[e]); }
    flat_pin(f.left); flat_pin(f.startAt);
    f.nextRef = X.myFlat[more ? f.next : f.nFrames - 1u];
}
template <class FD, uint32_t SET, bool ALLROWS = false>
struct FlatMid {
    FlatState2<FD>& f;
    __amdgpu_buffer_rsrc_t rsrc;
    bool has;
    template <class... T>
    __device__ __forceinline__ void operator()(T... firstHalf) const
    {
        using R = typename FD::R;
        (flat_pin(firstHalf), ...);
        if (ALLROWS || has) {
#pragma unroll
            for (int e = 0; e < FD::NE; ++e) {
                if (!(SET & (1u << e))) continue;
                const uint32_t off = f.idx[e];
                const flat_d2 v = __builtin_bit_cast(flat_d2, __builtin_amdgcn_raw_buffer_load_b128(rsrc, off, 0, 0));
                if (e < FD::NRES) {
                    f.rb[e < FD::NRES ? e : 0] = (R)v.x; f.rc[e < FD::NRES ? e : 0] = (R)v.y;
                    if (FD::ANTI0 && e == 0) f.ra[0] = (R)__builtin_bit_cast(double, __builtin_amdgcn_raw_buffer_load_b64(rsrc, off + 16u, 0, 0));
                } else {
                    const int g = e < FD::NRES ? 0 : e - FD::NRES;
                    f.cur[2 * g] = (R)v.x; f.cur[2 * g + 1] = (R)v.y;
                }
                f.idx[e] = off + f.stride[e];
            }
        }
    }
};
struct NoMid { template <class... T> __device__ __forceinline__ void operator()(T...) const {} };
template <int MODE, bool DERIVE, class R>
__device__ __forceinline__ ResPre<R> res_pre(R ra, R rb, R rc, R z1, R z2)
{
    ResPre<R> p;
    p.a = DERIVE ? (R)((R)1 - rb - rc) : ra;
    if (MODE == MODE_FAST || !std::is_same<R, double>::value) { p.p1 = rb; p.p2 = rc; }
    else { p.p1 = rb * z1; p.p2 = rc * z2; }
    return p;
}
template <int MODE, class R>
__device__ __forceinline__ R res_post(const ResPre<R>& p, R in, R& z1, R& z2)
{
    R y;
    if (MODE == MODE_FAST || !std::is_same<R, double>::value) y = dot3<MODE>(p.a, in, p.p1, z1, p.p2, z2);
    else y = p.a * in + p.p1 + p.p2;
    z2 = z1; z1 = y;
    return y;
}

template <class FD, int CH, class FBody, class FChunk, class FSync = BarrierSync>
__device__ __forceinline__ void flat2_loop(int depth, int nIter, int nChunks, int stampSlot, FlatState2<FD>& f, const StageCtx& X, const int* GE, FBody body, FChunk perChunk,
                                           const FSync& sync = FSync{})
{
#ifdef KLATT_STAMPS
    Stamps st;
#endif
    using R = typename FD::R;
    uint32_t staleG = 0;
    const __amdgpu_buffer_rsrc_t rsrc = __builtin_amdgcn_make_buffer_rsrc(const_cast<double2*>(X.A.track), 0, (int)X.A.trackBytes, 0x00020000);
    for (int iter = 0; iter < nIter; ++iter) {
        STAMP_BEGIN();
        STAMP_IDLE();
        const int c = iter - depth;
        const bool inRange = c >= 0 && c < nChunks;
        if (inRange) {
            sync.begin(c);
            const uint32_t t0 = (uint32_t)c * (uint32_t)CH, t1 = t0 + (uint32_t)CH;
            if (f.length <= t0) f.live = false;
            const bool busy = f.left > 0u || f.startAt <= t1;
// ... 57 lines not shown
                        if (tn == f.startAt) flat2_switch<FD>(f, X, GE);
                    }
                    const bool has = ALLROWS || f.left > 0u;
                    body(c, i, setTag, FlatMid<FD, SET, ALLROWS>{f, rsrc, has});
                    if (!ALLROWS && has) f.left--;
                }
                if (ALLROWS) f.left = f.left > (uint32_t)CH ? f.left - (uint32_t)CH : 0u;
            };
            constexpr uint32_t ALL = (1u << FD::NE) - 1u;
            const bool usual = FD::USUAL != 0u && FD::USUAL != ALL && c != 0 && (f.wmask & ~FD::USUAL) == 0u;
            const bool allRows = usual && __all(!f.live || (f.left >= (uint32_t)CH && f.startAt > t1));
            if (allRows) mixedChunk(std::integral_constant<uint32_t, FD::USUAL>{}, std::true_type{});
            else if (usual) mixedChunk(std::integral_constant<uint32_t, FD::USUAL>{}, std::false_type{});
            else mixedChunk(std::integral_constant<uint32_t, ALL>{}, std::false_type{});
            f.produced = f.length < t1 ? f.length : t1;
            perChunk();
        }
        STAMP_WORKED();
        if (inRange) sync.end(c); else sync.idle();
        STAMP_SYNCED();
    }
#ifdef KLATT_STAMPS
    if (X.A.debug && (threadIdx.x & (kLanes - 1)) == 0) {
        unsigned long long* o = X.A.debug + (blockIdx.x * 4 + stampSlot) * 8;
        o[0] = st.work; o[1] = st.wait; o[2] = st.n[0]; o[3] = st.n[1]; o[4] = st.n[2]; o[5] = st.c[0]; o[6] = st.c[1]; o[7] = st.c[2];
    }
#endif
    (void)stampSlot;
}

template <int MODE, bool NOISE, int CH, int WPS = KLATT_MINWAVES, bool NASAL = true, bool STREAM = false, bool FLAT = false, bool LONE = false>
__global__ void __launch_bounds__(kLanes * kStages, WPS) klatt_systolic(const KernelArgs A)
{
    static_assert(!LONE || STREAM, "LONE: a live handle pulled alone");
    static_assert(NASAL || !NOISE, "only quiet launches have a nasal-free instantiation");
    static_assert(NOISE || !STREAM, "live handles take the noisy instantiation");
    static_assert(!FLAT || (NOISE && !STREAM), "tracks: noisy batch launches");
    constexpr int SPLIT = stream_split<STREAM, WPS, LONE>();
    constexpr int MOVED = SPLIT & 3;
    using L = SysLds<NOISE, CH, FLAT, SPLIT>;
    static_assert(SPLIT != 3, "eight resonators in the head stage: not built");
    constexpr int kChunk = CH;
    extern __shared__ __attribute__((aligned(16))) unsigned char lds[];
    using PipeT = typename std::conditional<FLAT, sig_t, double>::type;
    PipeT* const pipeX = reinterpret_cast<PipeT*>(lds);
    PipeT* const pipeO = reinterpret_cast<PipeT*>(lds + L::kPipeO);
    PipeT* const pipeA = reinterpret_cast<PipeT*>(lds + L::kPipeO + L::kPipeBytes);
    PipeT* const pipeB = reinterpret_cast<PipeT*>(lds + L::kPipeO + (NOISE ? 2 : 1) * L::kPipeBytes);
    constexpr int nbuf_pipeX = L::kBufsX, nbuf_pipeO = L::kBufs, nbuf_pipeA = L::kBufs, nbuf_pipeB = L::kBufs;
    (void)nbuf_pipeX; (void)nbuf_pipeO; (void)nbuf_pipeA; (void)nbuf_pipeB;
    unsigned char* const tile = lds + L::kTileOff;
    long long* const rowBase = reinterpret_cast<long long*>(lds + L::kRowBase);
    uint32_t* const rowCount = reinterpret_cast<uint32_t*>(lds + L::kRowCount);
    uint32_t* const maxLenP = reinterpret_cast<uint32_t*>(lds + L::kMaxLen);

    const int lane = threadIdx.x & (kLanes - 1);
    const int wave = __builtin_amdgcn_readfirstlane(threadIdx.x >> 6);
    const long long slot = (long long)blockIdx.x * kLanes + lane;
    const uint32_t u = (slot < A.nSlots) ? A.order[slot] : 0xFFFFFFFFu;
    const bool live = (u != 0xFFFFFFFFu);

    UttDesc d;
    d.frameStart = 0; d.outStart = 0; d.nFrames = 0; d.seed = 0; d.flags = 0; d.length = 0;
    if (live) d = A.utt[u];
    const FrameWindow fw = frame_window(A, d);
    const StageCtx X{A, d, A.frames + fw.base * kNumParams, A.meta + fw.base, fw.off, fw.mask,
                     FLAT ? A.flatRef + d.frameStart : nullptr, FLAT ? A.sourceRef + d.frameStart : nullptr, LONE,
                     LONE ? reinterpret_cast<double*>(lds + L::kBytes + wave * kLoneLdsPerStage) : nullptr};
    const uint32_t nkey = noise_key(d.seed), ninc = noise_inc(d.seed), ninc2 = noise_inc2(ninc);
    constexpr int FINAL = NOISE ? 2 : 3;
#ifndef KLATT_PRELOAD
#define KLATT_PRELOAD 1
#endif
    constexpr bool kPre = !NOISE && KLATT_PRELOAD;

    uint32_t* const stageMaskP = maxLenP + 1;
    uint32_t* const syncP = reinterpret_cast<uint32_t*>(lds + L::kSync);
    if (threadIdx.x == 0) { *maxLenP = 0; *stageMaskP = 0; }
    if (threadIdx.x < 8) syncP[threadIdx.x] = 0;
    __syncthreads();
    int cand = wave;
    if (KLATT_PAIR && WPS == 2 && (NOISE || !NASAL)) {
        const uint32_t hw = __builtin_amdgcn_s_getreg((4 << 0) | (0 << 6) | (31 << 11));
        cand = (int)((((hw >> 4) & 3u) + ((hw & 1u) ? 2u : 0u)) & 3u);
    }
    if (wave == 0) atomicMax(maxLenP, d.length);
    if (lane == 0) atomicOr(stageMaskP, 1u << cand);
    __syncthreads();
    const int stage = __builtin_amdgcn_readfirstlane((*stageMaskP == 0xFu) ? cand : wave);
    if (stage == FINAL) { rowBase[lane] = d.outStart; rowCount[lane] = 0; }
    const uint32_t maxLen = *maxLenP;
    const int nChunks = (int)((maxLen + kChunk - 1) / kChunk);
    const int nIter = nChunks + (NOISE ? 2 : 3);
    const int fullChunks = STREAM ? (int)(A.maxSamples / (uint32_t)kChunk) : nChunks;
    double* const streamState = (STREAM && live) ? (A.statePtrs ? A.statePtrs[u] : A.state + (size_t)u * kStateDoubles) : nullptr;
    const bool streamPurge = STREAM && live && A.control && (A.control[u] & 1u);
#define PIPE(p, c, i) (p)[(((nbuf_##p) == 2 ? ((c) & 1) : ((c) % (nbuf_##p))) * kChunk + (i)) * kLanes + lane]
    using KSrc = LoopKnobs<false, (!NOISE || KLATT_NOISY_RUNS), false, STREAM, NOISE, KLATT_UNROLL, LONE, (STREAM && WPS == 1 && !LONE)>;
    using KFil = LoopKnobs<kPre, (!NOISE || KLATT_NOISY_RUNS), false, STREAM, NOISE, KLATT_UNROLL, LONE, (STREAM && WPS == 1 && !LONE)>;
    uint32_t noDelay = 0;
    auto never = [&]() __attribute__((always_inline)) { return false; };
    auto noBegin = [&](int) __attribute__((always_inline)) { return false; };
    auto noAlt = [&](int) __attribute__((always_inline)) {};
    auto noAltSample = [&](int, int, double) __attribute__((always_inline)) {};
    auto noFadeAlt = [&](int, bool, bool) __attribute__((always_inline)) { return false; };
    auto nothing = [&](int) __attribute__((always_inline)) {};
    auto noChunk = [&]() __attribute__((always_inline)) {};

    auto make_sync = [&](auto, auto, auto, int, int, int) __attribute__((always_inline)) { return BarrierSync{}; };
    using I0 = std::integral_constant<int, 0>; using I1 = std::integral_constant<int, 1>; using I2 = std::integral_constant<int, 2>;
    if (FLAT && KLATT_FLAT_SOURCE && stage == 0) {
        if constexpr (FLAT) {
#if KLATT_FLAT_LAYOUT == 2
            using FD = FlatDesc<0, 2, 5, true, 0, 0, double>;
            constexpr int GE[7] = {0, 1, 14, 20, 21, 22, 23};
            constexpr int CB = 2;
            constexpr uint32_t kUsualS0 = 0x67u, kAllS0 = 0x7Fu, kVibBit = 8u;
            constexpr bool kHead = true;
#else
            using FD = FlatDesc<0, 0, 4, false, 0, 0, double>;
            constexpr int GE[4] = {20, 21, 22, 23};
            constexpr int CB = 0;
            constexpr uint32_t kUsualS0 = 0xCu, kAllS0 = 0xFu, kVibBit = 1u;
            constexpr bool kHead = false;
#endif
            bool staleNP = false;
            FlatState2<FD> f;
            flat2_init<FD>(f, live, d, X, GE);
            PitchState ps;
            ps.cur0 = 0.0; ps.old0 = 0.0; ps.new0 = 0.0; ps.oldInc = 0.0; ps.newInc = 0.0;
            double pitchPhase = 0.0, vibPhase = 0.0, aspNoise = 0.0, invFade = 1.0, nfD = 1.0;
            uint32_t noiseSt = noise_first(nkey, ninc), cntF = 0, nfU = 0;
            uint32_t fadeEndAt = 0xFFFFFFFFu;
            int32_t lastIndex = -1;
            bool oldNull = true, newNull = false;
            SourceRef nextSrc{0.0, 0.0, 1.0, -1, 0u};
            if (live && d.nFrames > 0u) nextSrc = X.mySrc[0];
            auto source = [&](bool waveVib, auto setTag, const auto& mid) __attribute__((always_inline)) -> double {
                constexpr uint32_t SET = decltype(setTag)::value;
                double vib = 1.0;
                if (waveVib) {
                    const double vs = f.cur[CB + 1];
                    const double adv = frac_toward_zero(div_by(vs, A.sampleRateF, A.invSampleRate) + vibPhase);
                    vibPhase = (vs != 0.0) ? adv : vibPhase;
                    vib = (sin(vibPhase * 6.283185307179586) * 0.06 * f.cur[CB + 0]) + 1.0;
                }
                const double turbGain = f.cur[CB + 2], openQ = f.cur[CB + 3], voiceAmp = f.cur[CB + 4], aspAmp = f.cur[CB + 5], preGain = f.cur[CB + 6];
                pitchPhase = frac_toward_zero(div_by(ps.cur0 * vib, A.sampleRateF, A.invSampleRate) + pitchPhase);
                double voice = (pitchPhase * 2.0) - 1.0;
                aspNoise = noise_uniform(noiseSt) + 0.75 * aspNoise;
                noiseSt = noise_step2(noiseSt, ninc2);
                double asp = aspNoise * 0.2;
                double turb = asp * turbGain;
                turb = (pitchPhase >= openQ) ? turb : turb * 0.01;
                voice += turb;
                voice *= voiceAmp;
                asp *= aspAmp;
                const double src = asp + voice;
                const double out = (src * preGain) * 0.5;
                if constexpr (kHead) {
                    const ResPre<double> q0 = res_pre<MODE, false>(f.ra[0], f.rb[0], f.rc[0], f.z1[0], f.z2[0]);
                    const ResPre<double> q1 = res_pre<MODE, ((SET >> 1) & 1u) != 0u>(f.ra[1], f.rb[1], f.rc[1], f.z1[1], f.z2[1]);
                    const double caNP = f.cur[0];
                    mid(out, q0, q1, caNP);
                    double zin = f.z1[0];
                    const double n0 = res_post<MODE>(q0, out, zin, f.z2[0]);
                    f.z1[0] = out;
                    const double np = res_post<MODE>(q1, n0, f.z1[1], f.z2[1]);
                    return fade_value(out, np, caNP);
                } else {
                    mid(out);
                    return out;
                }
            };
            auto vib_live = [&]() __attribute__((always_inline)) -> bool { return f.cur[CB + 0] != 0.0 || f.cur[CB + 1] != 0.0 || vibPhase != vibPhase; };
            const __amdgpu_buffer_rsrc_t rsrc = __builtin_amdgcn_make_buffer_rsrc(const_cast<double2*>(A.track), 0, (int)A.trackBytes, 0x00020000);
#ifdef KLATT_STAMPS
            Stamps st;
#endif
            const auto sync = make_sync(std::integral_constant<int, L::kBufsX>{}, I0{}, I1{}, 0, 0, 0);
            for (int iter = 0; iter < nIter; ++iter) {
                STAMP_BEGIN();
                STAMP_IDLE();
                const int c = iter;
                int lastChunk = -1;
                if (c < nChunks) {
                    sync.begin(c);
                    lastChunk = c;
                    const uint32_t t0 = (uint32_t)c * (uint32_t)CH, t1 = t0 + (uint32_t)CH;
                    if (f.length <= t0) f.live = false;
                    const bool busy = f.left > 0u || f.startAt <= t1 || cntF < nfU || fadeEndAt < t1 || vib_live();
                    STAMP_KIND(__any(busy) ? -1 : 0);
                    if (!__any(busy)) {
                        uint32_t run = f.live ? (f.startAt - t0 - 1u) / (uint32_t)CH : 0xFFFFFFFFu;
#pragma unroll
                        for (int m = 32; m >= 1; m >>= 1) { const uint32_t o = (uint32_t)__shfl_xor((int)run, m, kLanes); run = o < run ? o : run; }
                        run = (uint32_t)__builtin_amdgcn_readfirstlane((int)run);
                        const uint32_t room = (uint32_t)(nChunks - c);
                        run = run < room ? run : room;
                        run = run < 1u ? 1u : run;
                        int cc = c;
                        if (kHead && staleNP) { f.ra[1] = 1.0 - f.rb[1] - f.rc[1]; staleNP = false; }
                        for (uint32_t q = 0; q < run; ++q) {
                            if (f.live) {
#pragma unroll
                                for (int i = 0; i < CH; ++i) { ps.cur0 += ps.oldInc; PIPE(pipeX, cc, i) = source(false, std::integral_constant<uint32_t, 0u>{}, NoMid{}); }
                                ps.old0 = ps.cur0;
                            }
                            if (q + 1 < run) { STAMP_WORKED(); sync.end(cc); STAMP_SYNCED(); STAMP_BEGIN(); ++iter; ++cc; sync.begin(cc); lastChunk = cc; }
                        }
                    } else {
                        auto mixedChunk = [&](auto setTag, auto allFadeTag) __attribute__((always_inline)) {
                        constexpr uint32_t SET = decltype(setTag)::value;
                        constexpr bool ALLFADE = decltype(allFadeTag)::value;
                        const bool vibChunk = (SET & kVibBit) != 0u || __any(vib_live());
                        staleNP = true;
#pragma unroll KLATT_MIX_UNROLL
                        for (int i = 0; i < CH; ++i) {
                            const uint32_t t = t0 + (uint32_t)i;
                            const bool deq = !ALLFADE && t + 1u == f.startAt;
                            if (!ALLFADE && __any(deq)) {
                                if (deq) {
                                    const SourceRef m = nextSrc;
                                    const uint32_t nf = f.nextRef.fadeSamples;
                                    newNull = (m.flags & FRAME_NULL) != 0;
                                    ps.new0 = newNull ? ps.cur0 : m.pitch;
                                    ps.newInc = newNull ? 0.0 : m.pitchInc;
                                    if (!newNull && oldNull) ps.old0 = m.pitch;
                                    oldNull = newNull;
                                    if (m.userIndex != -1) lastIndex = m.userIndex;
                                    nfD = (double)nf; nfU = nf;
                                    ps.new0 += ps.newInc * nfD;
                                    invFade = m.invFade;
                                    cntF = 0;
                                    fadeEndAt = t + nf + 1u;
                                    flat_pin(ps.new0); flat_pin(ps.newInc); flat_pin(ps.old0); flat_pin(invFade); flat_pin(lastIndex); flat_pin(oldNull);
                                    flat2_switch<FD>(f, X, GE);
                                    nextSrc = X.mySrc[f.next < f.nFrames ? f.next : f.nFrames - 1u];
                                }
                            }
                            if (ALLFADE) {
                                cntF++;
                                ps.cur0 = fade_value(ps.old0, ps.new0, div_by((double)cntF, nfD, invFade));
                            } else {
                            const bool fad = !deq && cntF < nfU;
                            const bool ending = !deq && !fad && t == fadeEndAt;
                            const bool glide = !deq && !fad && !ending;
                            const uint32_t cn = cntF + 1u;
                            const double ratio = div_by((double)cn, nfD, invFade);
                            const double fv = fade_value(ps.old0, ps.new0, ratio);
                            const double gv = ps.cur0 + ps.oldInc;
                            ps.cur0 = fad ? fv : (glide ? gv : ps.cur0);
                            ps.old0 = ending ? ps.new0 : (glide ? gv : ps.old0);
                            ps.oldInc = ending ? ps.newInc : ps.oldInc;
                            cntF = fad ? cn : cntF;
                            fadeEndAt = ending ? 0xFFFFFFFFu : fadeEndAt;
                            }
                            const bool waveVib = vibChunk && __any(vib_live());
                            const bool has = f.left > 0u;
                            PIPE(pipeX, c, i) = source(waveVib, setTag, FlatMid<FD, SET>{f, rsrc, has});
                            if (has) f.left--;
                        }
                        };
                        const bool usual = c != 0 && (f.wmask & ~kUsualS0) == 0u;
                        const bool allFade = usual && !__any(vib_live()) && __all(!f.live || (cntF + (uint32_t)CH <= nfU && f.startAt > t1));
                        if (allFade) mixedChunk(std::integral_constant<uint32_t, kUsualS0>{}, std::true_type{});
                        else if (usual) mixedChunk(std::integral_constant<uint32_t, kUsualS0>{}, std::false_type{});
                        else mixedChunk(std::integral_constant<uint32_t, kAllS0>{}, std::false_type{});
                    }
                }
                STAMP_WORKED();
                if (lastChunk >= 0) sync.end(lastChunk); else sync.idle();
                STAMP_SYNCED();
            }
#ifdef KLATT_STAMPS
            if (A.debug && lane == 0) {
                unsigned long long* o = A.debug + (blockIdx.x * 4 + 0) * 8;
                o[0] = st.work; o[1] = st.wait; o[2] = st.n[0]; o[3] = st.n[1]; o[4] = st.n[2]; o[5] = st.c[0]; o[6] = st.c[1]; o[7] = st.c[2];
            }
#endif
            if (live) {
                UttResult res;
                res.produced = d.length; res.framesTaken = f.next; res.lastIndex = lastIndex; res.drained = 1u;
                A.result[u] = res;
            }
        }
    } else if (stage == 0) {
        constexpr bool NP0 = (SPLIT >> 2) != 0;
        using D = StageDesc<NP0 ? 12 : 7, NP0 ? 2 : 0, 6, true, NP0, NP0>;
        constexpr int P[12] = {1, 2, 3, 4, 5, 6, 44, 13, 21, 14, 22, 23};
        constexpr int RF[2] = {7, 9}, RB[2] = {8, 10};
        StageFrame<D::NPARAM, D::NRES, true> f;
        PitchState ps;
        stage_frame_init(f, live, lds + L::kFrames, lane);
        ps.cur0 = 0.0; ps.old0 = 0.0; ps.new0 = 0.0; ps.oldInc = 0.0; ps.newInc = 0.0;
        double pitchPhase = 0.0, vibPhase = 0.0, aspNoise = 0.0;
        uint32_t noiseSt = noise_first(nkey, ninc);
        int32_t lastIndex = -1;
        bool vibFrames = false;
        constexpr int GR0[2] = {0, 1};
        if (STREAM && live) {
            if (streamState[239] != 0.0) {
                pitchPhase = streamState[208]; vibPhase = streamState[209]; aspNoise = streamState[210];
                lastIndex = (int32_t)streamState[220]; noiseSt = (uint32_t)streamState[221];
            }
            stage_state_load<D>(f, &ps, streamState, P, RF, RB, GR0, streamPurge);
            vibFrames = f.oldL[0] != 0.0 || f.oldL[kLanes] != 0.0 || f.getNew(0) != 0.0 || f.getNew(1) != 0.0;
        }

        auto source = [&](bool waveVib) __attribute__((always_inline)) -> double {
            double vib = 1.0;
            if (waveVib) {
                const double vs = f.cur[1];
                const double adv = frac_toward_zero(div_by(vs, A.sampleRateF, A.invSampleRate) + vibPhase);
                vibPhase = (vs != 0.0) ? adv : vibPhase;
                vib = (sin(vibPhase * 6.283185307179586) * 0.06 * f.cur[0]) + 1.0;
            }
            pitchPhase = frac_toward_zero(div_by(ps.cur0 * vib, A.sampleRateF, A.invSampleRate) + pitchPhase);
            double voice = (pitchPhase * 2.0) - 1.0;
            double src;
            if (NOISE) {
                aspNoise = noise_uniform(noiseSt) + 0.75 * aspNoise;
                noiseSt = noise_step2(noiseSt, ninc2);
                double asp = aspNoise * 0.2;
                double turb = asp * f.cur[2];
                turb = (pitchPhase >= f.cur[3]) ? turb : turb * 0.01;
                voice += turb;
                voice *= f.cur[4];
                asp *= f.cur[5];
                src = asp + voice;
            } else {
                src = voice * f.cur[4];
            }
            const double x = (src * f.cur[6]) * 0.5;
            if (!NP0) return x;
            const double n0 = dot3<MODE>(f.ra[0], x, f.rb[0], f.z1[0], f.rc[0], f.z2[0]);
            f.z2[0] = f.z1[0]; f.z1[0] = x;
            const double np = resonate<MODE>(f.z1[NP0 ? 1 : 0], f.z2[NP0 ? 1 : 0], f.ra[NP0 ? 1 : 0], f.rb[NP0 ? 1 : 0], f.rc[NP0 ? 1 : 0], n0);
            return fade_value(x, np, f.cur[NP0 ? 11 : 0]);
        };
        auto vib_live_now = [&]() __attribute__((always_inline)) -> bool {
            return vibFrames || f.cur[0] != 0.0 || f.cur[1] != 0.0 || vibPhase != vibPhase;
        };
        stage_loop<D, MODE, CH, KSrc>(0, nIter, nChunks, fullChunks, stage, f, &ps, &lastIndex, noDelay, P, RF, RB, X,
            [&]() __attribute__((always_inline)) { return __any(!f.done && vib_live_now()); },
            [&](int kind) __attribute__((always_inline)) -> bool { return !NOISE && kind == 0 && !__any(!f.done && ps.oldInc != 0.0); },
            [&](int c) __attribute__((always_inline)) {
                ps.cur0 += ps.oldInc;
                const double inc = div_by(ps.cur0 * 1.0, A.sampleRateF, A.invSampleRate);
                double ph[kChunk];
#pragma unroll
                for (int i = 0; i < kChunk; ++i) { pitchPhase = frac_toward_zero(inc + pitchPhase); ph[i] = pitchPhase; }
#pragma unroll
                for (int i = 0; i < kChunk; ++i) PIPE(pipeX, c, i) = ((((ph[i] * 2.0) - 1.0) * f.cur[4]) * f.cur[6]) * 0.5;
            },
            noAltSample,
            [&](int, int) __attribute__((always_inline)) { return 0.0; },
            [&](int c, int i, bool steady, double) __attribute__((always_inline)) {
                if (steady) ps.cur0 += ps.oldInc;
                PIPE(pipeX, c, i) = source(false);
            },
            [&](int c, bool lerp, bool gainOnly) __attribute__((always_inline)) -> bool {
                if (NOISE || !gainOnly) return false;
                constexpr int GI = 6;
                const double g0 = lerp ? f.oldL[GI * kLanes] : f.cur[GI], g1 = lerp ? f.getNew(GI) : f.cur[GI];
                if (__any(g1 != g1 || ps.new0 != ps.new0)) return false;
                const double gd = g1 - g0, p0 = ps.old0, pd = ps.new0 - p0, nf = (double)f.newFade;
                if (!__any(pd != 0.0 || p0 != p0)) {
// ... 15 lines not shown
                        const double ratio = div_by((double)f.cnt, nf, f.invFade);
                        ps.cur0 = p0 + (pd * ratio);
                        const double gain = g0 + (gd * ratio);
                        pitchPhase = frac_toward_zero(div_by(ps.cur0 * 1.0, A.sampleRateF, A.invSampleRate) + pitchPhase);
                        PIPE(pipeX, c, i) = ((((pitchPhase * 2.0) - 1.0) * f.cur[4]) * gain) * 0.5;
                        if (i == kChunk - 1) f.cur[GI] = gain;
                    }
                }
                return true;
            },
            [&](int c, int i, bool emit) __attribute__((always_inline)) {
                if (emit && f.hasNew && f.cnt == 0)
                    vibFrames = f.oldL[0] != 0.0 || f.oldL[kLanes] != 0.0 || f.getNew(0) != 0.0 || f.getNew(1) != 0.0;
                const bool waveVib = __any(emit && vib_live_now());
                if (emit) { PIPE(pipeX, c, i) = source(waveVib); f.produced++; }
            },
            [&](int n) __attribute__((always_inline)) { ps.old0 = ps.cur0; f.produced += n; },
            [&](int n) __attribute__((always_inline)) { f.produced += n; },
            noChunk);
        if (live) {
            UttResult res;
            res.produced = f.produced; res.framesTaken = f.nextFrame; res.lastIndex = lastIndex; res.drained = STREAM ? (f.done ? 1u : 0u) : 1u;
            A.result[u] = res;
        }
        if (STREAM && live) {
            stage_state_save<D>(f, &ps, streamState, P, GR0);
            streamState[208] = pitchPhase; streamState[209] = vibPhase; streamState[210] = aspNoise;
            streamState[220] = (double)lastIndex; streamState[221] = (double)noiseSt;
        }
    } else if (FLAT && stage == 1) {
        if constexpr (FLAT) {
#if KLATT_FLAT_LAYOUT == 2
            using FD = FlatDesc<1, 6, 0, false, 0x38u>;
            constexpr int GE[6] = {2, 3, 4, 5, 6, 7};
            FlatState2<FD> f;
            flat2_init<FD>(f, live, d, X, GE);
            flat2_loop<FD, CH>(1, nIter, nChunks, stage, f, X, GE,
                [&](int c, int i, auto setTag, const auto& mid) __attribute__((always_inline)) {
                    constexpr uint32_t SET = decltype(setTag)::value;
                    ResPre<sig_t> q[6];
#pragma unroll
                    for (int r = 0; r < 6; ++r) q[r] = ((SET >> r) & 1u) ? res_pre<MODE, true>(f.ra[r], f.rb[r], f.rc[r], f.z1[r], f.z2[r])
                                                                         : res_pre<MODE, false>(f.ra[r], f.rb[r], f.rc[r], f.z1[r], f.z2[r]);
                    mid(q[0], q[1], q[2], q[3], q[4], q[5]);
                    sig_t o = PIPE(pipeX, c, i);
#pragma unroll
                    for (int r = 0; r < 6; ++r) o = res_post<MODE>(q[r], o, f.z1[r], f.z2[r]);
                    PIPE(pipeO, c, i) = o;
                },
                noChunk, make_sync(std::integral_constant<int, L::kBufs>{}, I1{}, I1{}, 0, 0, 2));
#else
            using FD = FlatDesc<1, 6, 1, true, 0x63u>;
            constexpr int GE[7] = {0, 1, 2, 3, 4, 5, 14};
            FlatState2<FD> f;
            flat2_init<FD>(f, live, d, X, GE);
            flat2_loop<FD, CH>(1, nIter, nChunks, stage, f, X, GE,
                [&](int c, int i, auto setTag, const auto& mid) __attribute__((always_inline)) {
                    constexpr uint32_t SET = decltype(setTag)::value;
                    const ResPre<sig_t> q0 = res_pre<MODE, false>(f.ra[0], f.rb[0], f.rc[0], f.z1[0], f.z2[0]);
                    const ResPre<sig_t> q1 = res_pre<MODE, ((SET >> 1) & 1u) != 0u>(f.ra[1], f.rb[1], f.rc[1], f.z1[1], f.z2[1]);
                    const ResPre<sig_t> q2 = res_pre<MODE, ((SET >> 2) & 1u) != 0u>(f.ra[2], f.rb[2], f.rc[2], f.z1[2], f.z2[2]);
                    const ResPre<sig_t> q3 = res_pre<MODE, ((SET >> 3) & 1u) != 0u>(f.ra[3], f.rb[3], f.rc[3], f.z1[3], f.z2[3]);
                    const ResPre<sig_t> q4 = res_pre<MODE, ((SET >> 4) & 1u) != 0u>(f.ra[4], f.rb[4], f.rc[4], f.z1[4], f.z2[4]);
                    const ResPre<sig_t> q5 = res_pre<MODE, ((SET >> 5) & 1u) != 0u>(f.ra[5], f.rb[5], f.rc[5], f.z1[5], f.z2[5]);
                    const sig_t caNP = f.cur[0];
                    mid(q0, q1, q2, q3, q4, q5, caNP);
                    const sig_t x = PIPE(pipeX, c, i);
                    sig_t zin = f.z1[0];
                    const sig_t n0 = res_post<MODE>(q0, x, zin, f.z2[0]);
                    f.z1[0] = x;
                    const sig_t np = res_post<MODE>(q1, n0, f.z1[1], f.z2[1]);
                    sig_t o = fade_value(x, np, caNP);
                    o = res_post<MODE>(q2, o, f.z1[2], f.z2[2]);
                    o = res_post<MODE>(q3, o, f.z1[3], f.z2[3]);
                    o = res_post<MODE>(q4, o, f.z1[4], f.z2[4]);
                    o = res_post<MODE>(q5, o, f.z1[5], f.z2[5]);
                    PIPE(pipeO, c, i) = o;
                },
                noChunk);
#endif
        }
    } else if (FLAT && stage == 3) {
        if constexpr (FLAT) {
            using FD = FlatDesc<3, 4, 3, false, 0x77u>;
            constexpr int GE[7] = {8, 9, 10, 11, 17, 18, 19};
            FlatState2<FD> f;
            flat2_init<FD>(f, live, d, X, GE);
            sig_t fricNoise = 0;
            uint32_t noiseSt = noise_step(noise_first(nkey, ninc), ninc);
            flat2_loop<FD, CH>(1, nIter, nChunks, stage, f, X, GE,
                [&](int c, int i, auto setTag, const auto& mid) __attribute__((always_inline)) {
                    constexpr uint32_t SET = decltype(setTag)::value;
                    const ResPre<sig_t> q0 = res_pre<MODE, ((SET >> 0) & 1u) != 0u>(f.ra[0], f.rb[0], f.rc[0], f.z1[0], f.z2[0]);
                    const ResPre<sig_t> q1 = res_pre<MODE, ((SET >> 1) & 1u) != 0u>(f.ra[1], f.rb[1], f.rc[1], f.z1[1], f.z2[1]);
                    const ResPre<sig_t> q2 = res_pre<MODE, ((SET >> 2) & 1u) != 0u>(f.ra[2], f.rb[2], f.rc[2], f.z1[2], f.z2[2]);
                    const ResPre<sig_t> q3 = res_pre<MODE, ((SET >> 3) & 1u) != 0u>(f.ra[3], f.rb[3], f.rc[3], f.z1[3], f.z2[3]);
                    fricNoise = (sig_t)noise_uniform(noiseSt) + (sig_t)0.75 * fricNoise;
                    noiseSt = noise_step2(noiseSt, ninc2);
                    const sig_t fric = fricNoise * (sig_t)0.3 * f.cur[0];
                    const sig_t y = (fric * f.cur[1]) * (sig_t)0.5;
                    const sig_t pa1 = f.cur[2], pa2 = f.cur[3], pa3 = f.cur[4], pa4 = f.cur[5];
                    mid(q0, q1, q2, q3, y, pa1, pa2, pa3, pa4);
                    sig_t par = 0;
                    sig_t w = res_post<MODE>(q0, y, f.z1[0], f.z2[0]);
                    par += (w - y) * pa1;
                    w = res_post<MODE>(q1, y, f.z1[1], f.z2[1]);
                    par += (w - y) * pa2;
                    w = res_post<MODE>(q2, y, f.z1[2], f.z2[2]);
                    par += (w - y) * pa3;
                    w = res_post<MODE>(q3, y, f.z1[3], f.z2[3]);
                    par += (w - y) * pa4;
                    PIPE(pipeA, c, i) = y; PIPE(pipeB, c, i) = par;
                },
                noChunk, make_sync(std::integral_constant<int, L::kBufs>{}, I0{}, I1{}, 0, 0, 4));
        }
    } else if (FLAT && (KLATT_FLAT_EXHAUSTIVE || stage == 2)) {
        if constexpr (FLAT) {
#if KLATT_FLAT_LAYOUT == 2
            constexpr int GE[4] = {12, 13, 15, 16};
            using FD = FlatDesc<2, 2, 2, false, 0xEu>;
            constexpr int RS = 0;
#else
            constexpr int GE[6] = {6, 7, 12, 13, 15, 16};
            using FD = FlatDesc<2, 4, 2, false, 0x3Bu>;
            constexpr int RS = 2;
#endif
            FlatState2<FD> f;
            flat2_init<FD>(f, live, d, X, GE);
            int16_t* const myRow = reinterpret_cast<int16_t*>(tile + lane * kTileStride);
            uint32_t it = 0;
            auto flush_tile = [&](uint32_t tileStart, uint32_t validTo) __attribute__((always_inline)) {
                rowCount[lane] = f.produced;
                asm volatile("s_waitcnt lgkmcnt(0)" ::: "memory");
                constexpr int kChunksPerRow = kTile / 8;
                constexpr int kRowsPerPass = kLanes / kChunksPerRow;
                constexpr int kPasses = kLanes / kRowsPerPass;
                const int chunk = lane % kChunksPerRow;
                const uint32_t first = tileStart + (uint32_t)chunk * 8u;
                uint2 lo[kPasses], hi[kPasses];
                uint32_t cnt[kPasses];
                long long base[kPasses];
#pragma unroll
                for (int p = 0; p < kPasses; ++p) {
                    const int row = p * kRowsPerPass + lane / kChunksPerRow;
                    const uint2* src = reinterpret_cast<const uint2*>(tile + row * kTileStride + chunk * 16);
                    lo[p] = src[0]; hi[p] = src[1];
                    cnt[p] = rowCount[row];
                    base[p] = rowBase[row];
                }
#pragma unroll
                for (int p = 0; p < kPasses; ++p) {
                    if (cnt[p] > first && first < validTo) {
                        uint4* dst = reinterpret_cast<uint4*>(A.pcm + base[p] + first);
                        *dst = make_uint4(lo[p].x, lo[p].y, hi[p].x, hi[p].y);
                    }
                }
                asm volatile("s_waitcnt lgkmcnt(0)" ::: "memory");
            };
            flat2_loop<FD, CH>(2, nIter, nChunks, stage, f, X, GE,
                [&](int c, int i, auto setTag, const auto& mid) __attribute__((always_inline)) {
                    constexpr uint32_t SET = decltype(setTag)::value;
                    constexpr int NR = 2 + RS;
                    ResPre<sig_t> q[4];
#pragma unroll
                    for (int r = 0; r < NR; ++r) q[r] = ((SET >> r) & 1u) ? res_pre<MODE, true>(f.ra[r], f.rb[r], f.rc[r], f.z1[r], f.z2[r])
                                                                          : res_pre<MODE, false>(f.ra[r], f.rb[r], f.rc[r], f.z1[r], f.z2[r]);
                    const sig_t pa5 = f.cur[0], pa6 = f.cur[1], bypass = f.cur[2], outGain = f.cur[3];
                    if constexpr (RS == 2) mid(q[0], q[1], q[2], q[3], pa5, pa6, bypass, outGain);
                    else mid(q[0], q[1], pa5, pa6, bypass, outGain);
                    sig_t o = PIPE(pipeO, c, i);
                    const sig_t y = PIPE(pipeA, c, i);
#pragma unroll
                    for (int r = 0; r < RS; ++r) o = res_post<MODE>(q[r], o, f.z1[r], f.z2[r]);
                    sig_t par = PIPE(pipeB, c, i);
                    sig_t w = res_post<MODE>(q[RS], y, f.z1[RS], f.z2[RS]);
                    par += (w - y) * pa5;
                    w = res_post<MODE>(q[RS + 1], y, f.z1[RS + 1], f.z2[RS + 1]);
                    par += (w - y) * pa6;
                    par = fade_value(par, y, bypass);
                    const sig_t mix = o + par;
                    const sig_t v = (mix * outGain) * (sig_t)4000.0;
                    const sig_t lo = (v < (sig_t)32000.0) ? v : (sig_t)32000.0;
                    const sig_t cl = (lo > (sig_t)-32000.0) ? lo : (sig_t)-32000.0;
                    myRow[(it % kTile) + i] = (int16_t)(uint32_t)(int)cl;
                },
                [&]() __attribute__((always_inline)) { it += kChunk; if ((it % kTile) == 0) flush_tile(it - kTile, it); },
                make_sync(std::integral_constant<int, L::kBufs>{}, I2{}, I0{}, 2, 4, 0));
            if ((it % kTile) != 0) flush_tile(it - (it % kTile), it);
        }
    } else if (!NOISE && !NASAL && (stage == 1 || stage == 2)) {
        using D = StageDesc<6, 3, -1, false, false>;
        const bool s1 = (stage == 1);
        const int P[6] = {s1 ? 12 : 9, s1 ? 20 : 17, s1 ? 11 : 8, s1 ? 19 : 16, s1 ? 10 : 7, s1 ? 18 : 15};
        constexpr int RF[3] = {0, 2, 4}, RB[3] = {1, 3, 5};
        StageFrame<6, 3> f;
        stage_frame_init(f, live, lds + (s1 ? L::kFrames1 : L::kFrames2), lane);
        PipeT* const pin = s1 ? pipeX : pipeO;
// ... 190 lines not shown
```

nvspeechplayer_amd/speechPlayer.py:

```python
import math
from ctypes import POINTER, Structure, byref, c_double, c_int, c_short, c_void_p, cast
from ctypes import c_longlong as ctypes_longlong

import numpy as np

from . import _native

speechPlayer_frameParam_t = c_double

FRAME_FIELDS = [
    'voicePitch',
    'vibratoPitchOffset',
    'vibratoSpeed',
    'voiceTurbulenceAmplitude',
    'glottalOpenQuotient',
    'voiceAmplitude',
    'aspirationAmplitude',
    'cf1', 'cf2', 'cf3', 'cf4', 'cf5', 'cf6', 'cfN0', 'cfNP',
    'cb1', 'cb2', 'cb3', 'cb4', 'cb5', 'cb6', 'cbN0', 'cbNP',
    'caNP',
    'fricationAmplitude',
    'pf1', 'pf2', 'pf3', 'pf4', 'pf5', 'pf6',
    'pb1', 'pb2', 'pb3', 'pb4', 'pb5', 'pb6',
    'pa1', 'pa2', 'pa3', 'pa4', 'pa5', 'pa6',
# ... 1812 lines not shown
        sd = None if noiseSeed is None else np.ascontiguousarray(noiseSeed, dtype=np.uint32)
        self._check(self._dll.speechPlayer_batch_setText(self._h, n, ptrs, None if not espeakVoice else espeakVoice.encode("utf8"), float(speed),
                                                         pitch.ctypes.data, float(inflection), None if not voice else voice.encode("utf8"),
                                                         None if sd is None else sd.ctypes.data))
        self.nUtterances = n

    @property
    def totalSamples(self):
        return self._dll.speechPlayer_batch_totalSamples(self._h)

    @property
    def totalFrames(self):
        return self._dll.speechPlayer_batch_totalFrames(self._h)

    def utteranceSamples(self, u):
        return self._dll.speechPlayer_batch_utteranceSamples(self._h, u)

    def synthesize(self, wait=True):
        self._check(self._dll.speechPlayer_batch_synthesize(self._h))
        if wait:
            self._check(self._dll.speechPlayer_batch_wait(self._h))

    def wait(self):
        self._check(self._dll.speechPlayer_batch_wait(self._h))

    def read(self, u):
        n = self.utteranceSamples(u)
        buf = np.zeros(max(n, 1), dtype=np.int16)
        got = self._check(self._dll.speechPlayer_batch_read(self._h, u, buf.ctypes.data, n))
        return buf[:got]

    def readFloat(self, u):
        n = self.utteranceSamples(u)
        buf = np.zeros(max(n, 1), dtype=np.float32)
        got = self._check(self._dll.speechPlayer_batch_readFloat(self._h, u, buf.ctypes.data, n))
        return buf[:got]

    def writeWav(self, u, path):
        import wave
        pcm = self.read(u)
        with wave.open(path, "wb") as w:
            w.setnchannels(1); w.setsampwidth(2); w.setframerate(self.sampleRate)
            w.writeframes(pcm.astype("<i2").tobytes())

    def readAll(self, out=None):
        total = self.totalSamples
        if out is not None:
            if out.dtype != np.int16 or not out.flags["C_CONTIGUOUS"] or out.size < total:
                raise ValueError("readAll: out must be a contiguous int16 array of at least %d samples" % total)
            buf = out
        else:
            buf = np.empty(max(total, 1), dtype=np.int16)
        starts = np.zeros(self.nUtterances + 1, dtype=np.int64)
        got = self._check(self._dll.speechPlayer_batch_readAll(self._h, buf.ctypes.data, total, starts.ctypes.data))
        return buf[:got], starts

    def readAllAsync(self, out):
        total = self.totalSamples
        if out.dtype != np.int16 or not out.flags["C_CONTIGUOUS"] or out.size < total:
            raise ValueError("readAllAsync: out must be a contiguous int16 array of at least %d samples" % total)
        starts = np.zeros(self.nUtterances + 1, dtype=np.int64)
        got = self._check(self._dll.speechPlayer_batch_readAllAsync(self._h, out.ctypes.data, out.size, starts.ctypes.data))
        return out[:got], starts

    def readWait(self):
        self._check(self._dll.speechPlayer_batch_readWait(self._h))

    def digest(self, per_utterance=False):
        import ctypes
        whole = ctypes.c_ulonglong(0)
        per = np.zeros(max(self.nUtterances, 1), dtype=np.uint64) if per_utterance else None
        self._check(self._dll.speechPlayer_batch_digest(self._h, None if per is None else per.ctypes.data, ctypes.byref(whole)))
        return (int(whole.value), per[:self.nUtterances]) if per_utterance else int(whole.value)

    def getLastIndex(self, u):
        return self._dll.speechPlayer_batch_getLastIndex(self._h, u)

    def time(self, launches):
        ms = np.zeros(launches, dtype=np.float32)
        self._check(self._dll.speechPlayer_batch_time(self._h, launches, ms.ctypes.data))
        return ms

    def kernelInfo(self):
        info = np.zeros(20, dtype=np.int32)
        self._check(self._dll.speechPlayer_batch_kernelInfo(self._h, info.ctypes.data, len(info)))
        return dict(vgprs=int(info[0]), lds_bytes=int(info[1]), wavefronts=int(info[2]), cus=int(info[3]),
                    workgroups_per_cu_by_lds=int(info[4]), scratch_bytes=int(info[5]),
                    stage_parallel_chunk=int(info[6]), noisy_group=bool(info[7]),
                    lane_pipelined=bool(info[8]), lane_pipelined_utterances=int(info[9]),
                    nasal_free=bool(info[10]), nasal_free_utterances=int(info[11]),
                    tracked_utterances=int(info[12]), tracks=int(info[13]), track_mbytes=int(info[14]), tracked=bool(info[15]),
                    direct_utterances=int(info[16]), direct=bool(info[17]), direct_mbytes=int(info[18]))

    def devicePcm(self):
        return self._dll.speechPlayer_batch_devicePcm(self._h)

    def deviceOffset(self, u):
        return self._dll.speechPlayer_batch_deviceOffset(self._h, u)

    def close(self):
        if getattr(self, "_h", None):
            self._dll.speechPlayer_batch_destroy(self._h)
            self._h = None

    def __del__(self):
        try:
            self.close()
        except Exception:
            pass


class NodePlayer(object):

    def __init__(self, sampleRate, devices, mode=0, layout=None):
        self.sampleRate = sampleRate
        self._dll = _native.load()
        dev = np.ascontiguousarray(devices, dtype=np.int32)
        self._h = self._dll.speechPlayer_node_create(sampleRate, len(dev), dev.ctypes.data)
        if not self._h:
            raise RuntimeError("speechPlayer_node_create failed: %s" % _native.last_error())
        self._check(self._dll.speechPlayer_node_setOption(self._h, b"mode", mode))
        if layout is not None:
            self._check(self._dll.speechPlayer_node_setOption(self._h, b"layout", layout))
        self.nUtterances = 0
        self._lens = None

    def _check(self, rc):
        if rc is None or rc < 0:
            raise RuntimeError("speechPlayer node call failed: %s" % _native.last_error())
        return rc

    def setUtterances(self, frameStart, frames, minSamples, fadeSamples, userIndex=None, isNull=None, noiseSeed=None):
        fs = np.ascontiguousarray(frameStart, dtype=np.int64)
        fr = np.ascontiguousarray(frames, dtype=np.float64).reshape(-1, 47)
        m = np.ascontiguousarray(minSamples, dtype=np.uint32)
        f = np.ascontiguousarray(fadeSamples, dtype=np.uint32)
        assert fs[-1] == len(fr) == len(m) == len(f)
        ix = None if userIndex is None else np.ascontiguousarray(userIndex, dtype=np.int32)
        nu = None if isNull is None else np.ascontiguousarray(isNull, dtype=np.uint8)
        sd = None if noiseSeed is None else np.ascontiguousarray(noiseSeed, dtype=np.uint32)
        p = lambda a: None if a is None else a.ctypes.data
        self._check(self._dll.speechPlayer_node_setUtterances(self._h, len(fs) - 1, p(fs), p(fr), p(m), p(f), p(ix), p(nu), p(sd)))
        self.nUtterances = len(fs) - 1
        per = np.maximum(m.astype(np.int64), np.maximum(f.astype(np.int64), 1) + 1) + 1
        c = np.concatenate([[0], np.cumsum(per)])
        self._lens = c[fs[1:]] - c[fs[:-1]]

    def setIpa(self, texts, speed=1, basePitch=100, inflection=0.5, clauseType=None, noiseSeed=None, voice=None,
               trailing_silence_ms=150.0, textOf=None):
        from .ipa import _text_pointers, _clauses
        ptrs, n, keep = _text_pointers(texts, textOf)
        pitch = np.ascontiguousarray(np.broadcast_to(np.asarray(basePitch, dtype=np.float64), (n,)))
        sd = None if noiseSeed is None else np.ascontiguousarray(noiseSeed, dtype=np.uint32)
        by_name = voice is None or isinstance(voice, str)
        vo = None if by_name else np.ascontiguousarray(np.broadcast_to(np.asarray(voice, dtype=np.int32), (n,)))
        self._check(self._dll.speechPlayer_node_setIpa(self._h, int(self.sampleRate), n, ptrs.ctypes.data, float(speed), pitch.ctypes.data, float(inflection),
                                                       _clauses(clauseType, n), None if vo is None else vo.ctypes.data,
                                                       (voice.encode("utf8") if (by_name and voice) else None),
                                                       -1.0 if trailing_silence_ms is None else float(trailing_silence_ms), None if sd is None else sd.ctypes.data))
        del keep
        self.nUtterances = n
        self._lens = None

    def utteranceSamples(self, u):
        for d in range(self._dll.speechPlayer_node_devices(self._h)):
            mem = self.shardUtterances(d)
            at = np.flatnonzero(mem == u)
            if len(at):
                return self._dll.speechPlayer_batch_utteranceSamples(self._dll.speechPlayer_node_part(self._h, d), int(at[0]))
        raise RuntimeError("NodePlayer.utteranceSamples: utterance %d out of range" % u)

    @property
    def totalSamples(self):
        return self._dll.speechPlayer_node_totalSamples(self._h)

# ... 62 lines not shown
```

Measured before the change: 179.2 billion.

## Skip dead turbulence, aspiration and parallel-formant-1 terms per wavefront

Adds per-frame facts that record whether turbulence, aspiration or the first parallel resonator is ever nonzero. Each wavefront votes on these and dispatches to template-specialised source and parallel stages that drop the dead noise generation, turbulence mixing and the fourth parallel resonator. The aim is to cut FP64 arithmetic and register pressure in the tracked systolic path. In exchange the kernel gains more instantiations and code size, extra atomics for diagnostic counters, and an added tweak to the SIMD pairing selection.

```diff
diff --git a/nvspeechplayer_amd/csrc/klatt_batchplan.h b/nvspeechplayer_amd/csrc/klatt_batchplan.h
--- a/nvspeechplayer_amd/csrc/klatt_batchplan.h
+++ b/nvspeechplayer_amd/csrc/klatt_batchplan.h
@@ -44,7 +44,7 @@
     for (long long k = 0; k < n; ++k)
         if (!(meta[k].flags & FRAME_NULL)) fl |= facts[k].flags;
     const bool finite = !(fl & FACT_NONFINITE), needsNoise = (fl & FACT_NOISE) || !finite;
-    flags = needsNoise ? UTT_NEEDS_NOISE : (!(fl & FACT_NASAL) ? UTT_NO_NASAL : 0u);
+    flags = (needsNoise ? UTT_NEEDS_NOISE : (!(fl & FACT_NASAL) ? UTT_NO_NASAL : 0u)) | (fl & kUttPresent);
     shape = finite ? (!(fl & FACT_UNBOUNDED) ? 3 : 1) : 0;
 }
 
@@ -264,4 +264,22 @@
     return p;
 }
 
-}
+template <class FlagsOf>
+inline void dead_wave_counts(const uint32_t* order, long long first, long long n, FlagsOf flagsOf, int built, long long counts[3], int width = kLanes)
+{
+    counts[0] = counts[1] = counts[2] = 0;
+    for (long long w = first; w < first + n; w += width) {
+        uint32_t present = 0;
+        bool any = false;
+        for (long long s = w; s < std::min(w + width, first + n); ++s)
+            if (order[s] != kNoUtt) { present |= flagsOf(order[s]); any = true; }
+        if (!any) continue;
+        const bool noTurb = !(present & UTT_TURBULENCE), noAsp = noTurb && !(present & UTT_ASPIRATION);
+        const int body = ((built & 4) && noAsp) ? 2 : (((built & 2) && noTurb) ? 1 : 0);
+        counts[0] += ((built & 1) && !(present & UTT_PARALLEL1)) ? 1 : 0;
+        counts[1] += body >= 1 ? 1 : 0;
+        counts[2] += body >= 2 ? 1 : 0;
+    }
+}
+
+}
diff --git a/nvspeechplayer_amd/csrc/klatt_consts.h b/nvspeechplayer_amd/csrc/klatt_consts.h
--- a/nvspeechplayer_amd/csrc/klatt_consts.h
+++ b/nvspeechplayer_amd/csrc/klatt_consts.h
@@ -11,11 +11,18 @@
 constexpr uint32_t UTT_NO_NASAL = 2u;
 constexpr uint32_t UTT_TRACKED = 4u;
 constexpr uint32_t UTT_DIRECT = 8u;
+constexpr uint32_t UTT_TURBULENCE = 16u;
+constexpr uint32_t UTT_ASPIRATION = 32u;
+constexpr uint32_t UTT_PARALLEL1 = 64u;
+constexpr uint32_t kUttPresent = UTT_TURBULENCE | UTT_ASPIRATION | UTT_PARALLEL1;
 constexpr int kUttKindShift = 8;
 
 constexpr uint32_t FACT_NOISE = 1u;
 constexpr uint32_t FACT_NONFINITE = 2u;
 constexpr uint32_t FACT_NASAL = 4u;
 constexpr uint32_t FACT_UNBOUNDED = 8u;
+constexpr uint32_t FACT_TURBULENCE = UTT_TURBULENCE;
+constexpr uint32_t FACT_ASPIRATION = UTT_ASPIRATION;
+constexpr uint32_t FACT_PARALLEL1 = UTT_PARALLEL1;
 
 }
diff --git a/nvspeechplayer_amd/csrc/klatt_device.h b/nvspeechplayer_amd/csrc/klatt_device.h
--- a/nvspeechplayer_amd/csrc/klatt_device.h
+++ b/nvspeechplayer_amd/csrc/klatt_device.h
@@ -100,6 +100,8 @@
     double negPiOverSr;
     double twoPiOverSr;
     unsigned long long* debug;
+    uint32_t* deadWaves;
+    uint32_t deadTerms;
 };
 
 __device__ constexpr int kResF[kNumRes] = {13, 14, 12, 11, 10, 9, 8, 7, 25, 26, 27, 28, 29, 30};
diff --git a/nvspeechplayer_amd/csrc/klatt_engine.hip b/nvspeechplayer_amd/csrc/klatt_engine.hip
--- a/nvspeechplayer_amd/csrc/klatt_engine.hip
+++ b/nvspeechplayer_amd/csrc/klatt_engine.hip
@@ -519,6 +519,9 @@
     hipStream_t side[6] = {nullptr, nullptr, nullptr, nullptr, nullptr, nullptr};
     hipEvent_t forkEvent = nullptr, join[6] = {nullptr, nullptr, nullptr, nullptr, nullptr, nullptr};
     int quietLast = 1;
+    int deadTerms = 1;
+    DeviceBuffer<uint32_t> dDeadWaves;
+    long long planDeadWaves[3] = {0, 0, 0};
     long long nUtt = 0, nFrames = 0, nSlots = 0;
     long long nLists = 0, nFramesSpoken = 0;
     std::vector<long long> uttFrameStart;
@@ -866,16 +869,19 @@
         t.negPiOverSr = a.negPiOverSr; t.twoPiOverSr = a.twoPiOverSr;
         const long long tg = b->nJobs;
         if (tg > 0x7FFFFFFF) { set_error("too many tracks: %lld", b->nJobs); return -1; }
+        if (b->dDeadWaves.reserve(3)) return -1;
+        HIP_TRY(hipMemsetAsync(b->dDeadWaves.ptr, 0, 3 * sizeof(uint32_t), st));
         hipLaunchKernelGGL(klatt_tracks, dim3((unsigned)tg), dim3(kLanes * kTrackWaves), 0, st, t);
         HIP_TRY(hipGetLastError());
         a.order = b->dOrder.ptr + b->nQuiet; a.nSlots = nTr;
         a.flatRef = b->dFlatRef.ptr; a.sourceRef = b->dSourceRef.ptr; a.track = b->dTrack.ptr;
         a.trackBytes = (uint32_t)std::min<unsigned long long>(((unsigned long long)b->trackEntries + kTrackPad) * sizeof(double2), 0xFFFFFFFFull);
+        a.deadWaves = b->dDeadWaves.ptr; a.deadTerms = b->deadTerms ? kUttPresent : 0u;
         const GroupPlan pl = plan_group(b->layout, true, b->nSlots, nTr + nNoisy, b->cus);
         const long long g = (nTr + kLanes - 1) / kLanes;
         if (pl.chunk == 8 ? launch_systolic<true, KLATT_FLAT_CH, KLATT_FLAT_WPS, true, false, true>(a, b->mode, g, st)
                           : launch_systolic<true, 16, 1, true, false, true>(a, b->mode, g, st)) return -1;
-        a.flatRef = nullptr; a.sourceRef = nullptr; a.track = nullptr;
+        a.flatRef = nullptr; a.sourceRef = nullptr; a.track = nullptr; a.deadWaves = nullptr; a.deadTerms = 0u;
     }
     if (nDir > 0) {
         hipStream_t st = next_stream();
@@ -1900,7 +1906,7 @@
     b->dDense.release(); b->dDenseStart.release(); b->dFacts.release(); b->hFacts.release();
     b->dRecords.release(); b->dShapeTable.release(); b->dRep.release(); b->dMismatch.release();
     b->dFrames.release(); b->dMeta.release(); b->dUtt.release(); b->dOrder.release(); b->dPcm.release(); b->dResult.release();
-    b->dFloat.release(); b->dDebug.release(); b->dDigest.release(); b->bounce.release();
+    b->dFloat.release(); b->dDebug.release(); b->dDigest.release(); b->bounce.release(); b->dDeadWaves.release();
     b->dFlatRef.release(); b->dSourceRef.release(); b->dJobs.release(); b->dShapes.release(); b->dTrack.release();
     b->dDirectJobs.release(); b->dDirectFirst.release(); b->dDirectHdr.release(); b->dDirectRec.release();
     delete b;
@@ -1920,6 +1926,7 @@
     if (!strcmp(name, "quiet_last")) { b->quietLast = value ? 1 : 0; return 0; }
     if (!strcmp(name, "layout")) { b->layout = value < 0 ? -1 : (value > 2 ? 1 : value); return 0; }
     if (!strcmp(name, "tracks")) { b->tracks = value ? 1 : 0; return 0; }
+    if (!strcmp(name, "dead_terms")) { b->deadTerms = value ? 1 : 0; return 0; }
     if (!strcmp(name, "track_budget_mb")) { b->trackBudgetMB = value < 0 ? 0 : value; return 0; }
     if (!strcmp(name, "direct")) { b->direct = value < 0 ? 0 : (value > 2 ? 2 : value); return 0; }
     if (!strcmp(name, "direct_lean")) { b->directLean = value < 0 ? -1 : (value ? 1 : 0); return 0; }
@@ -2568,6 +2575,7 @@
     b->nNoNasalUtt = lanes.nNoNasal;
     b->nQuiet = lanes.nQuietSlots; b->nNoNasal = lanes.nNoNasalSlots;
     b->nTracked = lanes.nTrackedUtt > 0 ? lanes.nTracked : 0; b->nTrackedUtt = lanes.nTrackedUtt;
+    dead_wave_counts(lanes.order.data(), lanes.nQuietSlots, b->nTracked, [&](uint32_t u) { return c.utt[u].flags; }, KLATT_DEAD_TERMS, b->planDeadWaves);
     b->nJobs = lanes.nTrackedUtt > 0 ? (long long)c.plan.jobs.size() : 0; b->trackEntries = lanes.nTrackedUtt > 0 ? (long long)c.plan.entries : 0;
     b->nDirect = c.nDirectUtt > 0 ? lanes.nDirectSlots : 0; b->nDirectUtt = c.nDirectUtt; b->nDirectFrames = (long long)c.scratch.directJobs.size();
     b->directAligned = c.nDirectUtt > 0 && c.directAligned;
@@ -3391,6 +3399,16 @@
         info[18] = (int)std::min<long long>(b->nDirectFrames * (long long)(kDirectEntries * sizeof(double2) + kDirectStages * sizeof(DirectHdr)) >> 20, 0x7FFFFFFF);
         info[19] = 0;
     }
+    if (nInfo >= 23) {
+        uint32_t dead[3] = {0u, 0u, 0u};
+        if (b->launched && nTr > 0 && b->dDeadWaves.ptr) {
+            HIP_TRY(hipStreamSynchronize(b->stream));
+            HIP_TRY(hipMemcpy(dead, b->dDeadWaves.ptr, sizeof dead, hipMemcpyDeviceToHost));
+        } else if (nTr > 0 && b->deadTerms) {
+            for (int k = 0; k < 3; ++k) dead[k] = (uint32_t)std::min<long long>(b->planDeadWaves[k], 0x7FFFFFFFll);
+        }
+        for (int k = 0; k < 3; ++k) info[20 + k] = (int)std::min<uint32_t>(dead[k], 0x7FFFFFFFu);
+    }
     return 0;
 }
 
@@ -3489,8 +3507,11 @@
     if (nFrames < 0 || (nFrames > 0 && (!frames || !facts24)) || sampleRate <= 0) { set_error("frameFacts: bad arguments"); return -1; }
     const double maxBw = 690.0 * sampleRate / M_PI, maxF = 9900.0 * sampleRate / (2.0 * M_PI);
     FrameFacts* const out = static_cast<FrameFacts*>(facts24);
+    constexpr uint32_t kRouting = FACT_NOISE | FACT_NONFINITE | FACT_NASAL | FACT_UNBOUNDED;
     if (!onDevice) {
-        parallel_ranges(nFrames, 1 << 13, [&](long long a, long long e) { for (long long k = a; k < e; ++k) out[k] = frame_facts(reinterpret_cast<const double*>(frames + k), maxF, maxBw); });
+        parallel_ranges(nFrames, 1 << 13, [&](long long a, long long e) {
+            for (long long k = a; k < e; ++k) { out[k] = frame_facts(reinterpret_cast<const double*>(frames + k), maxF, maxBw); out[k].flags &= kRouting; }
+        });
         return nFrames;
     }
     if (nFrames == 0) return 0;
@@ -3503,6 +3524,7 @@
     hipLaunchKernelGGL(klatt_frame_facts, dim3(grid), dim3(256), 0, nullptr, dF.ptr, dO.ptr, nFrames, maxF, maxBw);
     HIP_TRY(hipGetLastError());
     HIP_TRY(hipMemcpy(out, dO.ptr, (size_t)nFrames * sizeof(FrameFacts), hipMemcpyDeviceToHost));
+    for (long long k = 0; k < nFrames; ++k) out[k].flags &= kRouting;
     return nFrames;
 }
 
diff --git a/nvspeechplayer_amd/csrc/klatt_plan.h b/nvspeechplayer_amd/csrc/klatt_plan.h
--- a/nvspeechplayer_amd/csrc/klatt_plan.h
+++ b/nvspeechplayer_amd/csrc/klatt_plan.h
@@ -22,6 +22,12 @@
     unsigned long long w;
     memcpy(&w, &v, 8);
     return (w & 0x7FF0000000000000ull) != 0x7FF0000000000000ull;
+}
+KLATT_LAYOUT_HD inline bool fact_plus_zero(double v)
+{
+    unsigned long long w;
+    memcpy(&w, &v, 8);
+    return w == 0ull;
 }
 KLATT_LAYOUT_HD inline double fact_abs(double v) { return v < 0 ? -v : v; }
 KLATT_LAYOUT_HD constexpr unsigned long long fact_key(int n)
@@ -60,6 +66,10 @@
     if (p[23] != 0.0 || !(p[21] >= 1.0) || !(p[22] >= 0.0) || !(p[21] <= 1e6) || !(p[22] <= 1e6) ||
         !(fact_abs(p[13]) <= 1e6) || !(fact_abs(p[14]) <= 1e6) || !(fact_abs(p[5]) <= 1e30) || !(fact_abs(p[44]) <= 1e30))
         fl |= 4u;
+    if (!fact_plus_zero(p[3])) fl |= FACT_TURBULENCE;
+    if (!fact_plus_zero(p[6])) fl |= FACT_ASPIRATION;
+    if (p[37] != 0.0 || !(p[31] >= 1.0) || !(p[31] <= 1e6) || !(fact_abs(p[25]) <= 1e6) || !(fact_abs(p[24]) <= 1e30) || !(fact_abs(p[44]) <= 1e30))
+        fl |= FACT_PARALLEL1;
     bool inRange = true;
     for (int i = 7; i <= 14; ++i) inRange = inRange && (fact_abs(p[i]) <= maxF) && (p[i + 8] >= 0.0) && (p[i + 8] <= maxBw);
     for (int i = 25; i <= 30; ++i) inRange = inRange && (fact_abs(p[i]) <= maxF) && (p[i + 6] >= 0.0) && (p[i + 6] <= maxBw);
diff --git a/nvspeechplayer_amd/csrc/klatt_systolic.h b/nvspeechplayer_amd/csrc/klatt_systolic.h
--- a/nvspeechplayer_amd/csrc/klatt_systolic.h
+++ b/nvspeechplayer_amd/csrc/klatt_systolic.h
@@ -31,6 +31,9 @@
 #define KLATT_FLAT_EXHAUSTIVE 1
 #endif
 constexpr int kStages = 4;
+#ifndef KLATT_DEAD_TERMS
+#define KLATT_DEAD_TERMS 3
+#endif
 #ifndef KLATT_FLAT_SOURCE
 #define KLATT_FLAT_SOURCE 1
 #endif
@@ -744,13 +747,13 @@
     (void)stampSlot;
 }
 
-template <int STAGE_, int NRES_, int NGAIN_, bool ANTI0_, uint32_t USUAL_ = 0, uint32_t USUAL2_ = 0, class R_ = sig_t>
+template <int STAGE_, int NRES_, int NGAIN_, bool ANTI0_, uint32_t USUAL_ = 0, uint32_t USUAL2_ = 0, class R_ = sig_t, uint32_t SKIP_ = 0>
 struct FlatDesc {
     using R = R_;
     static constexpr int STAGE = STAGE_;
     static constexpr int NRES = NRES_, NGAIN = NGAIN_, NE = NRES_ + NGAIN_;
     static constexpr bool ANTI0 = ANTI0_;
-    static constexpr uint32_t USUAL = USUAL_, USUAL2 = USUAL2_;
+    static constexpr uint32_t USUAL = USUAL_, USUAL2 = USUAL2_, SKIP = SKIP_;
 };
 
 struct BarrierSync {
@@ -816,6 +819,11 @@
     uint32_t moving = 0, still = 0;
 #pragma unroll
     for (int e = 0; e < FD::NE; ++e) {
+        if constexpr (FD::SKIP != 0u) {
+#pragma unroll
+            for (int k = 0; k < kTrackEntries; ++k)
+                if (((FD::SKIP >> k) & 1u) && k < GE[e] && (e == 0 || k > GE[e - 1])) { const bool mv = (p.mask >> k) & 1u; moving += mv ? 1u : 0u; still += mv ? 0u : 1u; }
+        }
         const bool moves = (p.mask >> GE[e]) & 1u;
         f.idx[e] = (part + (moves ? hdr + moving : still)) * 16u;
         f.stride[e] = moves ? nMove * 16u : 0u;
@@ -1039,7 +1047,8 @@
     int cand = wave;
     if (KLATT_PAIR && WPS == 2 && (NOISE || !NASAL)) {
         const uint32_t hw = __builtin_amdgcn_s_getreg((4 << 0) | (0 << 6) | (31 << 11));
-        cand = (int)((((hw >> 4) & 3u) + ((hw & 1u) ? 2u : 0u)) & 3u);
+        const uint32_t simd = (hw >> 4) & 3u, odd = hw & 1u;
+        cand = (int)(KLATT_PAIR == 2 ? (simd ^ odd) : KLATT_PAIR == 3 ? (simd ^ (odd ? 3u : 0u)) : ((simd + (odd ? 2u : 0u)) & 3u));
     }
     if (wave == 0) atomicMax(maxLenP, d.length);
     if (lane == 0) atomicOr(stageMaskP, 1u << cand);
@@ -1063,24 +1072,39 @@
     auto noFadeAlt = [&](int, bool, bool) __attribute__((always_inline)) { return false; };
     auto nothing = [&](int) __attribute__((always_inline)) {};
     auto noChunk = [&]() __attribute__((always_inline)) {};
+    uint32_t deadSet = 0;
+    if (FLAT) {
+        const uint32_t mine = live ? d.flags : 0u;
+#pragma unroll
+        for (uint32_t bit = UTT_TURBULENCE; bit <= UTT_PARALLEL1; bit <<= 1) deadSet |= __any((mine & bit) != 0u) ? 0u : bit;
+        deadSet = (uint32_t)__builtin_amdgcn_readfirstlane((int)(deadSet & A.deadTerms));
+    }
 
     auto make_sync = [&](auto, auto, auto, int, int, int) __attribute__((always_inline)) { return BarrierSync{}; };
     using I0 = std::integral_constant<int, 0>; using I1 = std::integral_constant<int, 1>; using I2 = std::integral_constant<int, 2>;
     if (FLAT && KLATT_FLAT_SOURCE && stage == 0) {
         if constexpr (FLAT) {
+            auto sourceStage = [&](auto deadTag) __attribute__((always_inline)) {
+            constexpr int DEAD = decltype(deadTag)::value;
+            constexpr bool NOTURB = DEAD >= 1;
 #if KLATT_FLAT_LAYOUT == 2
-            using FD = FlatDesc<0, 2, 5, true, 0, 0, double>;
-            constexpr int GE[7] = {0, 1, 14, 20, 21, 22, 23};
+            using FD = FlatDesc<0, 2, NOTURB ? 4 : 5, true, 0, 0, double, NOTURB ? (1u << 21) : 0u>;
+            constexpr int GE[7] = {0, 1, 14, 20, NOTURB ? 22 : 21, NOTURB ? 23 : 22, 23};
             constexpr int CB = 2;
-            constexpr uint32_t kUsualS0 = 0x67u, kAllS0 = 0x7Fu, kVibBit = 8u;
+            constexpr uint32_t kUsualS0 = NOTURB ? 0x37u : 0x67u, kAllS0 = NOTURB ? 0x3Fu : 0x7Fu, kVibBit = 8u;
             constexpr bool kHead = true;
 #else
-            using FD = FlatDesc<0, 0, 4, false, 0, 0, double>;
-            constexpr int GE[4] = {20, 21, 22, 23};
+            using FD = FlatDesc<0, 0, NOTURB ? 3 : 4, false, 0, 0, double, NOTURB ? (1u << 21) : 0u>;
+            constexpr int GE[4] = {20, NOTURB ? 22 : 21, NOTURB ? 23 : 22, 23};
             constexpr int CB = 0;
-            constexpr uint32_t kUsualS0 = 0xCu, kAllS0 = 0xFu, kVibBit = 1u;
+            constexpr uint32_t kUsualS0 = NOTURB ? 0x6u : 0xCu, kAllS0 = NOTURB ? 0x7u : 0xFu, kVibBit = 1u;
             constexpr bool kHead = false;
 #endif
+            constexpr int CA = CB + (NOTURB ? 2 : 4);
+            if (A.deadWaves && lane == 0) {
+                if (DEAD >= 1) atomicAdd(A.deadWaves + 1, 1u);
+                if (DEAD >= 2) atomicAdd(A.deadWaves + 2, 1u);
+            }
             bool staleNP = false;
             FlatState2<FD> f;
             flat2_init<FD>(f, live, d, X, GE);
@@ -1102,17 +1126,24 @@
                     vibPhase = (vs != 0.0) ? adv : vibPhase;
                     vib = (sin(vibPhase * 6.283185307179586) * 0.06 * f.cur[CB + 0]) + 1.0;
                 }
-                const double turbGain = f.cur[CB + 2], openQ = f.cur[CB + 3], voiceAmp = f.cur[CB + 4], aspAmp = f.cur[CB + 5], preGain = f.cur[CB + 6];
+                const double voiceAmp = f.cur[CA + 0], aspAmp = f.cur[CA + 1], preGain = f.cur[CA + 2];
+                (void)aspAmp; (void)aspNoise; (void)noiseSt;
                 pitchPhase = frac_toward_zero(div_by(ps.cur0 * vib, A.sampleRateF, A.invSampleRate) + pitchPhase);
                 double voice = (pitchPhase * 2.0) - 1.0;
-                aspNoise = noise_uniform(noiseSt) + 0.75 * aspNoise;
-                noiseSt = noise_step2(noiseSt, ninc2);
-                double asp = aspNoise * 0.2;
-                double turb = asp * turbGain;
-                turb = (pitchPhase >= openQ) ? turb : turb * 0.01;
-                voice += turb;
+                double asp = 0.0;
+                if constexpr (DEAD < 2) {
+                    aspNoise = noise_uniform(noiseSt) + 0.75 * aspNoise;
+                    noiseSt = noise_step2(noiseSt, ninc2);
+                    asp = aspNoise * 0.2;
+                }
+                if constexpr (!NOTURB) {
+                    const double turbGain = f.cur[CB + 2], openQ = f.cur[CB + 3];
+                    double turb = asp * turbGain;
+                    turb = (pitchPhase >= openQ) ? turb : turb * 0.01;
+                    voice += turb;
+                }
                 voice *= voiceAmp;
-                asp *= aspAmp;
+                if constexpr (DEAD < 2) asp *= aspAmp;
                 const double src = asp + voice;
                 const double out = (src * preGain) * 0.5;
                 if constexpr (kHead) {
@@ -1241,6 +1272,10 @@
                 res.produced = d.length; res.framesTaken = f.next; res.lastIndex = lastIndex; res.drained = 1u;
                 A.result[u] = res;
             }
+            };
+            if ((KLATT_DEAD_TERMS & 4) && (deadSet & (UTT_TURBULENCE | UTT_ASPIRATION)) == (UTT_TURBULENCE | UTT_ASPIRATION)) sourceStage(std::integral_constant<int, 2>{});
+            else if ((KLATT_DEAD_TERMS & 2) && (deadSet & UTT_TURBULENCE)) sourceStage(std::integral_constant<int, 1>{});
+            else sourceStage(std::integral_constant<int, 0>{});
         }
     } else if (stage == 0) {
         constexpr bool NP0 = (SPLIT >> 2) != 0;
@@ -1422,10 +1457,14 @@
         }
     } else if (FLAT && stage == 3) {
         if constexpr (FLAT) {
-            using FD = FlatDesc<3, 4, 3, false, 0x77u>;
-            constexpr int GE[7] = {8, 9, 10, 11, 17, 18, 19};
+            auto parallel = [&](auto noP1Tag) __attribute__((always_inline)) {
+            constexpr bool NOP1 = decltype(noP1Tag)::value;
+            constexpr int NR = NOP1 ? 3 : 4;
+            using FD = FlatDesc<3, NR, 3, false, NOP1 ? 0x3Bu : 0x77u, 0, sig_t, NOP1 ? (1u << 8) : 0u>;
+            constexpr int GE[7] = {NOP1 ? 9 : 8, NOP1 ? 10 : 9, NOP1 ? 11 : 10, NOP1 ? 17 : 11, NOP1 ? 18 : 17, NOP1 ? 19 : 18, 19};
             FlatState2<FD> f;
             flat2_init<FD>(f, live, d, X, GE);
+            if (NOP1 && A.deadWaves && lane == 0) atomicAdd(A.deadWaves + 0, 1u);
             sig_t fricNoise = 0;
             uint32_t noiseSt = noise_step(noise_first(nkey, ninc), ninc);
             flat2_loop<FD, CH>(1, nIter, nChunks, stage, f, X, GE,
@@ -1434,25 +1473,40 @@
                     const ResPre<sig_t> q0 = res_pre<MODE, ((SET >> 0) & 1u) != 0u>(f.ra[0], f.rb[0], f.rc[0], f.z1[0], f.z2[0]);
                     const ResPre<sig_t> q1 = res_pre<MODE, ((SET >> 1) & 1u) != 0u>(f.ra[1], f.rb[1], f.rc[1], f.z1[1], f.z2[1]);
                     const ResPre<sig_t> q2 = res_pre<MODE, ((SET >> 2) & 1u) != 0u>(f.ra[2], f.rb[2], f.rc[2], f.z1[2], f.z2[2]);
-                    const ResPre<sig_t> q3 = res_pre<MODE, ((SET >> 3) & 1u) != 0u>(f.ra[3], f.rb[3], f.rc[3], f.z1[3], f.z2[3]);
+                    constexpr int R3 = NR - 1;
+                    ResPre<sig_t> q3{};
+                    if constexpr (!NOP1) q3 = res_pre<MODE, ((SET >> 3) & 1u) != 0u>(f.ra[R3], f.rb[R3], f.rc[R3], f.z1[R3], f.z2[R3]);
                     fricNoise = (sig_t)noise_uniform(noiseSt) + (sig_t)0.75 * fricNoise;
                     noiseSt = noise_step2(noiseSt, ninc2);
                     const sig_t fric = fricNoise * (sig_t)0.3 * f.cur[0];
                     const sig_t y = (fric * f.cur[1]) * (sig_t)0.5;
                     const sig_t pa1 = f.cur[2], pa2 = f.cur[3], pa3 = f.cur[4], pa4 = f.cur[5];
-                    mid(q0, q1, q2, q3, y, pa1, pa2, pa3, pa4);
-                    sig_t par = 0;
-                    sig_t w = res_post<MODE>(q0, y, f.z1[0], f.z2[0]);
-                    par += (w - y) * pa1;
-                    w = res_post<MODE>(q1, y, f.z1[1], f.z2[1]);
-                    par += (w - y) * pa2;
-                    w = res_post<MODE>(q2, y, f.z1[2], f.z2[2]);
-                    par += (w - y) * pa3;
-                    w = res_post<MODE>(q3, y, f.z1[3], f.z2[3]);
-                    par += (w - y) * pa4;
-                    PIPE(pipeA, c, i) = y; PIPE(pipeB, c, i) = par;
+                    if constexpr (NOP1) {
+                        mid(q0, q1, q2, y, pa2, pa3, pa4);
+                        sig_t w = res_post<MODE>(q0, y, f.z1[0], f.z2[0]);
+                        sig_t par = (w - y) * pa2;
+                        w = res_post<MODE>(q1, y, f.z1[1], f.z2[1]);
+                        par += (w - y) * pa3;
+                        w = res_post<MODE>(q2, y, f.z1[2], f.z2[2]);
+                        par += (w - y) * pa4;
+                        PIPE(pipeA, c, i) = y; PIPE(pipeB, c, i) = par;
+                    } else {
+                        mid(q0, q1, q2, q3, y, pa1, pa2, pa3, pa4);
+                        sig_t par = 0;
+                        sig_t w = res_post<MODE>(q0, y, f.z1[0], f.z2[0]);
+                        par += (w - y) * pa1;
+                        w = res_post<MODE>(q1, y, f.z1[1], f.z2[1]);
+                        par += (w - y) * pa2;
+                        w = res_post<MODE>(q2, y, f.z1[2], f.z2[2]);
+                        par += (w - y) * pa3;
+                        w = res_post<MODE>(q3, y, f.z1[R3], f.z2[R3]);
+                        par += (w - y) * pa4;
+                        PIPE(pipeA, c, i) = y; PIPE(pipeB, c, i) = par;
+                    }
                 },
                 noChunk, make_sync(std::integral_constant<int, L::kBufs>{}, I0{}, I1{}, 0, 0, 4));
+            };
+            if ((KLATT_DEAD_TERMS & 1) && (deadSet & UTT_PARALLEL1)) parallel(std::true_type{}); else parallel(std::false_type{});
         }
     } else if (FLAT && (KLATT_FLAT_EXHAUSTIVE || stage == 2)) {
         if constexpr (FLAT) {
diff --git a/nvspeechplayer_amd/speechPlayer.py b/nvspeechplayer_amd/speechPlayer.py
--- a/nvspeechplayer_amd/speechPlayer.py
+++ b/nvspeechplayer_amd/speechPlayer.py
@@ -1918,15 +1918,16 @@
         return ms
 
     def kernelInfo(self):
-        info = np.zeros(20, dtype=np.int32)
+        info = np.zeros(23, dtype=np.int32)
         self._check(self._dll.speechPlayer_batch_kernelInfo(self._h, info.ctypes.data, len(info)))
+        dead = dict(waves_without_parallel1=int(info[20]), waves_without_turbulence=int(info[21]), waves_without_aspiration=int(info[22]))
         return dict(vgprs=int(info[0]), lds_bytes=int(info[1]), wavefronts=int(info[2]), cus=int(info[3]),
                     workgroups_per_cu_by_lds=int(info[4]), scratch_bytes=int(info[5]),
                     stage_parallel_chunk=int(info[6]), noisy_group=bool(info[7]),
                     lane_pipelined=bool(info[8]), lane_pipelined_utterances=int(info[9]),
                     nasal_free=bool(info[10]), nasal_free_utterances=int(info[11]),
                     tracked_utterances=int(info[12]), tracks=int(info[13]), track_mbytes=int(info[14]), tracked=bool(info[15]),
-                    direct_utterances=int(info[16]), direct=bool(info[17]), direct_mbytes=int(info[18]))
+                    direct_utterances=int(info[16]), direct=bool(info[17]), direct_mbytes=int(info[18]), **dead)
 
     def devicePcm(self):
         return self._dll.speechPlayer_batch_devicePcm(self._h)
```

Result: faster. 189.9 billion (median of 6 runs) (+6.0%).
